# eladb3/SViT

Hardware: AMD Instinct MI355X
Metric: clips/sec (fwd+bwd) SViT 16x224^2 bf16 (higher is better)
Workload: dtype bf16; 1 GPU; SViT 16x224^2, 8 clips/GPU, 4 object tokens/frame, fwd+CE+bwd+clip+AdamW; global_batch=8, parallelism=dp1, ranks_seen=1, forced_dp=False, launch=hip-graph replay, input=fp32 clips, resident in the replayed step's input buffers, hip_library=svit_amd/lib/libsvit_hip.so

## Files before the change

### include/svit_hip.h

```cpp
#ifndef SVIT_HIP_H
#define SVIT_HIP_H
#include <stdint.h>
#ifdef __cplusplus
extern "C" {
#endif

#define SVIT_HEAD_DIM 96

int svit_version(void);
const char* svit_arch(void);

enum {
  SVIT_EPI_BF16 = 0,
  SVIT_EPI_GELU = 1,
  SVIT_EPI_RESID = 2,
  SVIT_EPI_F32 = 3,
  SVIT_EPI_DGELU = 4,
  SVIT_EPI_RELQ = 5
};
typedef struct {
  const void* A; int32_t lda;
  const void* W; int32_t ldw;
  const float* bias;
  void* out; int32_t ldo;
// ... 80 lines not shown
  int32_t stride_hw;
  int32_t mode;
  float eps;
  float out_scale;
  const void* relq_R; const int32_t* relq_map; int32_t relq_lpad; float relq_scale;
} svit_pool_args;
int svit_pool_ln_fwd(const svit_pool_args* a, void* stream);

typedef struct {
  const void* d_main; int32_t main_is_f32; int32_t ld_main;
  const void* d_res; const void* d_extra;
  const void* pre; const float* mean; const float* rstd; const float* gamma;
  void* dpre; float* dgamma; float* dbeta;
  int32_t B, heads, Nout;
  float* workspace; int64_t workspace_floats;
  int32_t main_parts; int64_t main_part_stride;
  int32_t extra_is_bf16;
} svit_pool_ln_bwd_args;
int svit_pool_ln_bwd(const svit_pool_ln_bwd_args* a, void* stream);
typedef struct {
  const void* dpre; const float* conv_w; void* dqkv; int32_t which;
  int32_t B, heads, T, H, W, n_obj, stride_hw;
} svit_pool_dgrad_args;
typedef struct {
  const void* dpre; const void* qkv; int32_t which; float* dw;
  int32_t B, heads, T, H, W, n_obj, stride_hw;
  float* workspace; int64_t workspace_floats;
} svit_pool_wgrad_args;
int svit_pool_ln_fwd_qkv(const svit_pool_args* args3, void* stream);
int svit_pool_weight_sel(const float* src_base, const int64_t* src_off, uint32_t* dst, int n_tables,
                         void* stream);
int svit_pool_ln_fwd_qkv_sel(const svit_pool_args* args3, const uint32_t* const* sel3, void* stream);
int svit_pool_ln_bwd_qkv(const svit_pool_ln_bwd_args* args3, void* stream);
#ifdef SVIT_DIAG_POOL_STREAMING
int svit_pool_conv_dgrad(const svit_pool_dgrad_args* a, void* stream);
int svit_pool_conv_wgrad(const svit_pool_wgrad_args* a, void* stream);
int svit_pool_conv_dgrad_qkv(const svit_pool_dgrad_args* args3, void* stream);
int svit_pool_conv_wgrad_qkv(const svit_pool_wgrad_args* args3, void* stream);
#endif
int svit_pool_conv_bwd_qkv(const svit_pool_dgrad_args* dgrad3, const svit_pool_wgrad_args* wgrad3,
                           void* stream);
int64_t svit_pool_conv_bwd_workspace(const svit_pool_dgrad_args* dgrad3);

typedef struct {
  void* qa; int32_t ld;
  const float* rel_h; const float* rel_w; const float* rel_t;
  const int32_t* idx_h; const int32_t* idx_w; const int32_t* idx_t;
  int32_t B, heads, qt, qh, qw, kt, kh, kw, n_obj;
  float inv_scale;
} svit_relq_args;
int svit_relpos_q_fwd(const svit_relq_args* a, void* stream);
typedef struct {
  const void* qa; const void* dqa; int32_t ld;
  const float* rel_h; const float* rel_w; const float* rel_t;
  const int32_t* idx_h; const int32_t* idx_w; const int32_t* idx_t;
  float* dq_extra;
  float* drel_h; float* drel_w; float* drel_t;
  int32_t rows_h, rows_w, rows_t;
  int32_t B, heads, qt, qh, qw, kt, kh, kw, n_obj;
  float inv_scale;
  float* workspace; int64_t workspace_floats;
} svit_relq_bwd_args;
int svit_relpos_q_bwd(const svit_relq_bwd_args* a, void* stream);
typedef struct {
  const void* P; int32_t ldp; void* qa; int32_t ld;
  const int32_t* idx_h; const int32_t* idx_w; const int32_t* idx_t;
  int32_t row_h, row_w, row_t;
  int32_t B, heads, qt, qh, qw, kt, kh, kw, n_obj;
  float inv_scale;
} svit_relq_gather_args;
int svit_relpos_gather(const svit_relq_gather_args* a, void* stream);
typedef struct {
  const void* dqa; int32_t ld; void* D; int32_t ldd;
  const int32_t* idx_h; const int32_t* idx_w; const int32_t* idx_t;
  int32_t off_h, off_w, off_t;
  int32_t B, heads, qt, qh, qw, kt, kh, kw, n_obj;
  float inv_scale;
} svit_relq_scatter_args;
int svit_relpos_scatter(const svit_relq_scatter_args* a, void* stream);

typedef struct {
  const void* qa; const void* ka; const void* v; void* ctx; float* lse2;
  int32_t B, heads, Nq, Nk, DA; float scale; int32_t bias_cols;
} svit_attn_fwd_args;
int svit_attn_fwd(const svit_attn_fwd_args* a, void* stream);
typedef struct {
  const void* qa; const void* ka; const void* v; const void* ctx; const void* dctx;
  const float* lse2; float* delta;
  void* dqa;
  float* dk; float* dv;
  int32_t B, heads, Nq, Nk, DA, q_splits; float scale;
  int32_t bias_cols;
  void* relD; int32_t relD_ld; const int32_t* relD_map; float relD_scale;
  const void* relR; float* relX;
} svit_attn_bwd_args;
int svit_attn_bwd(const svit_attn_bwd_args* a, void* stream);
int svit_attn_bwd_parts(const svit_attn_bwd_args* a);

int svit_maxpool_fwd(const float* x, float* y, uint8_t* idx, int B, int T, int H, int W,
                     int n_obj, int C, void* stream);
int svit_maxpool_bwd(const float* dy, const uint8_t* idx, float* dx, int B, int T, int H, int W,
                     int n_obj, int C, void* stream);
int svit_maxpool_bwd_bf16(const float* dy, const uint8_t* idx, void* dx_bf16, int B, int T, int H, int W,
                          int n_obj, int C, void* stream);

int svit_sumsq(const float* g, int64_t n, float* sumsq, float* workspace,
               int64_t workspace_floats, void* stream);
int svit_adamw_step(float* p, const float* g, float* m, float* v, int64_t n, const float* sumsq,
                    float max_norm, float lr, float beta1, float beta2, float eps, float wd,
                    int step, float grad_scale, void* stream);

typedef struct {
  float lr[2], weight_decay[2];
  float max_norm, clip_value, grad_scale, reserved;
} svit_step_host;
typedef struct {
  int64_t applied, skipped;
  int32_t consecutive, apply;
  float coef, bc1, bc2_sqrt, sumsq, grad_norm, reserved;
} svit_step_dev;

int svit_adamw_bias_table(float beta1, float beta2, float* table, int64_t capacity, int64_t* n_entries);

int svit_step_guard(const float* g, int64_t n, const svit_step_host* host_rec, svit_step_dev* dev_rec,
                    const float* bias_table, int64_t table_entries, float* workspace, int64_t workspace_floats,
                    void* stream);
int svit_adamw_step_guarded(float* p, const float* g, float* m, float* v, int64_t n, int64_t n_decay,
                            const svit_step_host* host_rec, const svit_step_dev* dev_rec, float beta1, float beta2,
                            float eps, void* stream);

typedef struct {
  const float* tokens; int32_t B, N, C, T, O;
  const float* keep;
  const float* w_proj; const float* b_proj; int32_t n_cls;
  const float* w_box; const float* b_box;
  const float* w_bce; const float* b_bce;
  const float* w_con; const float* b_con;
  float* logits; float* boxes; float* contact; float* xobj;
} svit_head_args;
int svit_head_fwd(const svit_head_args* a, void* stream);
typedef struct {
  svit_head_args f;
  const float* dlogits; const float* dboxes; const float* dcontact; const float* dxobj;
  float* dtokens;
  float* gw_proj; float* gb_proj; float* gw_box; float* gb_box; float* gw_bce; float* gb_bce; float* gw_con; float* gb_con;
  int32_t ordered;
} svit_head_bwd_args;
int svit_head_bwd(const svit_head_bwd_args* g, void* stream);

int svit_haog_loss(const float* pred, const float* tar, const float* contact,
                   const int64_t* contact_tar, float* losses, float* g_l1, float* g_bce,
                   float* g_giou, float* g_contact, int R, int Rc, void* stream);
int svit_haog_loss_bwd(const float* upstream, const float* g_l1, const float* g_bce,
                       const float* g_giou, const float* g_contact, float* dpred,
                       float* dcontact, int R, int Rc, void* stream);

int svit_ce_loss(const float* logits, const int64_t* labels, int B, int C, float* loss, float* dlogits, void* stream);
int svit_ce_loss_soft(const float* logits, const float* target, const int64_t* labels, const void* mix, float on,
                      float off, int B, int C, float* loss, float* dlogits, void* stream);
int svit_step_draws(uint64_t* state, const float* keep, int n_blocks, int per_block, float* scales,
                    int n_drop, float p_drop, float* drop, void* stream);

int svit_ensemble_update(const float* preds, const int64_t* labels, const int64_t* clip_ids,
                         int N, int C, int num_clips, int num_videos, int mode, int repeat,
                         float* video_preds, int64_t* video_labels, int64_t* clip_count,
                         int* err, void* stream);
int svit_topk_correct(const float* video_preds, const int64_t* video_labels, int V, int C,
                      const int* ks, int nk, int* counts, int* err, void* stream);
int svit_debug_set(int key, int val);
int svit_debug_set_tn(int step_us_x100, int atomic_tbs_x100);
int svit_debug_set_tn_tile(int mode);
int svit_debug_set_pool(int key, int val);
int svit_debug_pool_bwd_path(void);
int svit_attn_debug_set(int key, int val);
int svit_debug_reset(void);
#ifdef __cplusplus
}
// ... 3 lines not shown
```

### svit_amd/csrc/attn_bwd.hip

```cpp
#include <algorithm>
#include "attn_common.h"
#include "../../include/svit_hip.h"

#ifdef SVIT_ATTN_STAMPS
__device__ unsigned long long g_bwd_stamps[64];
extern "C" int svit_debug_attn_bwd_stamps(unsigned long long* host, int n) {
  return (int)hipMemcpyFromSymbol(host, HIP_SYMBOL(g_bwd_stamps), sizeof(unsigned long long) * n);
}
#define BSTAMP(slot)                                                                    \
  do {                                                                                  \
    __builtin_amdgcn_sched_barrier(0);                                                  \
    if (stamp_on) g_bwd_stamps[(slot)] = wall_clock64();                                \
    __builtin_amdgcn_sched_barrier(0);                                                  \
  } while (0)
#else
#define BSTAMP(slot) do {} while (0)
#endif

#ifndef SVIT_ATTN_QSTAGE
#define SVIT_ATTN_QSTAGE 1
#endif

namespace {
using namespace attn;
constexpr int KT = 64;
constexpr int QR = 64;
constexpr float LN2 = 0.6931471805599453f;

struct FragAddr {
  unsigned rowa[2], tra[2];
  __device__ __forceinline__ void init(unsigned base, int lane) {
    const int hh = lane >> 5, row = lane & 31, sw = (row >> 2) & 3;
    rowa[0] = base + row * 64 + 16 * ((0 + hh) ^ sw);
    rowa[1] = base + row * 64 + 16 * ((2 + hh) ^ sw);
    const int cg = (lane >> 4) & 1, i = lane & 15, q = i >> 2, pp = i & 3;
    const int r0 = 4 * hh, ch = 2 * cg + (pp >> 1);
    const unsigned tb = base + 8 * (pp & 1);
    tra[0] = tb + (r0 + q) * 64 + 16 * (ch ^ ((r0 >> 2) & 3));
    tra[1] = tb + (r0 + 8 + q) * 64 + 16 * (ch ^ (((r0 + 8) >> 2) & 3));
  }
};

template <int DA, int KSU>
__global__ __launch_bounds__(256, 2) void attn_bwd_dq_kernel(svit_attn_bwd_args a) {
#if __HIP_DEVICE_COMPILE__
  constexpr int NP = DA / 32;
  constexpr int K_BYTES = KT * DA * 2, V_BYTES = KT * HD * 2, STAGE = K_BYTES + V_BYTES;
  using KLoad = BufTile<KT, DA, 4>;
  using VLoad = BufTile<KT, HD, 4>;
  extern __shared__ __attribute__((aligned(16))) unsigned char smem[];
  const int tid = threadIdx.x, lane = tid & 63, wave = tid >> 6, hh = lane >> 5;
#ifdef SVIT_ATTN_STAMPS
  const bool stamp_on = blockIdx.x == 0 && blockIdx.y == 0 && tid == 0;
#endif
  BSTAMP(0);
  const int wgid = xcd_remap(blockIdx.y * gridDim.x + blockIdx.x, gridDim.x * gridDim.y);
  const int bh = wgid / gridDim.x, b = bh / a.heads, head = bh % a.heads;
  const int qtile = wgid % gridDim.x;
  const int q0 = qtile * 128 + wave * 32;
  const int qi = q0 + (lane & 31);
  const int qc = min(qi, a.Nq - 1);
  const bf16_t* qa = (const bf16_t*)a.qa + ((size_t)bh * a.Nq) * DA;
  const bf16_t* ka = (const bf16_t*)a.ka + ((size_t)bh * a.Nk) * DA;
  const bf16_t* vv = (const bf16_t*)a.v + ((size_t)bh * a.Nk) * HD;
  const bf16_t* dor = (const bf16_t*)a.dctx + ((size_t)b * a.Nq + qc) * a.heads * HD + head * HD;
  const float lse = a.lse2[(size_t)bh * a.Nq + qc];

  const int nt = (a.Nk + KT - 1) / KT;
  KLoad kload;
  VLoad vload;
  kload.init(DA, wave, lane);
  vload.init(HD, wave, lane);
  const auto krs = __builtin_amdgcn_make_buffer_rsrc((void*)ka, 0, a.Nk * DA * 2, 0x00020000);
  const auto vrs = __builtin_amdgcn_make_buffer_rsrc((void*)vv, 0, a.Nk * HD * 2, 0x00020000);
  auto issue = [&](int t) {
    unsigned char* st = smem + (t & 1) * STAGE;
    const unsigned k0 = (unsigned)t * KT;
    kload.issue_auto(krs, k0 * DA * 2u, DA, a.Nk - (int)k0, st, wave, lane);
    vload.issue_auto(vrs, k0 * HD * 2u, HD, a.Nk - (int)k0, st + K_BYTES, wave, lane);
  };
  BSTAMP(1);
  issue(0);
  BSTAMP(2);

  bf16x8_t qf[KSU], dof[6];
#pragma unroll
  for (int ks = 0; ks < 6; ++ks) dof[ks] = *(const bf16x8_t*)(dor + ks * 16 + hh * 8);
  using QStage = RowStage<DA>;
  if constexpr (SVIT_ATTN_QSTAGE != 0) {
    unsigned char* qreg = smem + STAGE + wave * QStage::BYTES;
    QStage::issue(qa, DA, q0, a.Nq, qreg, lane);
    wait_vmcnt<0>();
#pragma unroll
    for (int ks = 0; ks < KSU; ++ks) qf[ks] = QStage::frag(qreg, ks, lane);
  } else {
#pragma unroll
    for (int ks = 0; ks < KSU; ++ks) qf[ks] = *(const bf16x8_t*)(qa + (size_t)qc * DA + ks * 16 + hh * 8);
  }
  float dlt;
  {
    const bf16_t* orow = (const bf16_t*)a.ctx + ((size_t)b * a.Nq + qc) * a.heads * HD + head * HD;
    float part = 0.f;
#pragma unroll
    for (int ks = 0; ks < 6; ++ks) {
      const uint4 o = *(const uint4*)(orow + ks * 16 + hh * 8);
      const uint4 d = __builtin_bit_cast(uint4, dof[ks]);
      uint4 q = __builtin_bit_cast(uint4, qf[ks]);
      if (qc == 0) q = make_uint4(0, 0, 0, 0);
      part += lo_bf16(d.x) * (lo_bf16(o.x) - lo_bf16(q.x)) + hi_bf16(d.x) * (hi_bf16(o.x) - hi_bf16(q.x));
      part += lo_bf16(d.y) * (lo_bf16(o.y) - lo_bf16(q.y)) + hi_bf16(d.y) * (hi_bf16(o.y) - hi_bf16(q.y));
      part += lo_bf16(d.z) * (lo_bf16(o.z) - lo_bf16(q.z)) + hi_bf16(d.z) * (hi_bf16(o.z) - hi_bf16(q.z));
      part += lo_bf16(d.w) * (lo_bf16(o.w) - lo_bf16(q.w)) + hi_bf16(d.w) * (hi_bf16(o.w) - hi_bf16(q.w));
    }
    dlt = part + __shfl_xor(part, 32, 64);
    if (hh == 0 && qi < a.Nq) {
      float* sc = a.delta + (size_t)bh * a.Nq * 2;
      sc[qi] = -lse;
      sc[a.Nq + qi] = -dlt;
    }
  }

#pragma unroll
  for (int ks = 0; ks < KSU; ++ks) asm volatile("" : "+v"(qf[ks]));
#pragma unroll
  for (int ks = 0; ks < 6; ++ks) asm volatile("" : "+v"(dof[ks]));
  float lse_p = lse, dlt_p = dlt;
  asm volatile("" : "+v"(lse_p), "+v"(dlt_p));

  f32x16_t dq[NP];
#pragma unroll
  for (int j = 0; j < NP; ++j)
#pragma unroll
    for (int r = 0; r < 16; ++r) dq[j][r] = 0.f;

  FragAddr fa;
  fa.init((unsigned)(size_t)smem, lane);
  constexpr bool CINIT = DA == 128;
  f32x16_t s_init, dp_init;
#pragma unroll
  for (int r = 0; r < 16; ++r) { s_init[r] = CINIT ? -lse_p : 0.f; dp_init[r] = CINIT ? -dlt_p : 0.f; }

  static_prio(blockIdx.y * gridDim.x + blockIdx.x, wave, 4);
  BSTAMP(3);
  for (int t = 0; t < nt; ++t) {
// ... 147 lines not shown
    bf16_t vals[NV];
#pragma unroll
    for (int it = 0; it < NV; ++it) {
      const int e = it * 64 + lane, rl = e / EXTRA, j = e % EXTRA;
      vals[it] = *(const bf16_t*)(ost + rl * OROW + (96 + j) * 2);
    }
    asm volatile("s_waitcnt lgkmcnt(0)" ::: "memory");
    const int ldd = a.relD_ld, cpr = ldd >> 3;
    const int rpp = ldd <= 128 ? 32 : 8;
    bf16_t* Dg = (bf16_t*)a.relD + ((size_t)bh * a.Nq) * ldd;
    for (int r0 = 0; r0 < 32; r0 += rpp) {
      const int n16 = rpp * cpr;
      for (int i = lane; i < n16; i += 64) *(uint4*)(ost + i * 16) = make_uint4(0u, 0u, 0u, 0u);
      asm volatile("s_waitcnt lgkmcnt(0)" ::: "memory");
#pragma unroll
      for (int it = 0; it < NV; ++it) {
        const int e = it * 64 + lane, rl = e / EXTRA, j = e % EXTRA;
        if (rl >= r0 && rl < r0 + rpp && cols[it] >= 0)
          *(bf16_t*)(ost + ((rl - r0) * ldd + cols[it]) * 2) = f32_to_bf16(bf16_to_f32(vals[it]) * a.relD_scale);
      }
      asm volatile("s_waitcnt lgkmcnt(0)" ::: "memory");
      for (int i = lane; i < n16; i += 64) {
        const int rl = i / cpr, ch = i % cpr;
        if (q0 + r0 + rl < a.Nq)
          *(uint4*)(Dg + (size_t)(q0 + r0 + rl) * ldd + ch * 8) = *(const uint4*)(ost + i * 16);
      }
      if (a.relX && rpp == 32) {
        f32x16_t ex[3];
#pragma unroll
        for (int pb = 0; pb < 3; ++pb)
#pragma unroll
          for (int r = 0; r < 16; ++r) ex[pb][r] = 0.f;
        const bf16_t* R = (const bf16_t*)a.relR;
        for (int ks = 0; ks < ldd / 16; ++ks) {
          const bf16x8_t dfrag = *(const bf16x8_t*)(ost + ((lane & 31) * ldd + 16 * ks + 8 * hh) * 2);
#pragma unroll
          for (int pb = 0; pb < 3; ++pb) {
            const bf16x8_t rfrag = *(const bf16x8_t*)(R + (size_t)(pb * 32 + (lane & 31)) * ldd + 16 * ks + 8 * hh);
            ex[pb] = mfma32(rfrag, dfrag, ex[pb]);
          }
        }
        if (qi < a.Nq) {
          float* xr = a.relX + ((size_t)bh * a.Nq + qi) * HD;
#pragma unroll
          for (int pb = 0; pb < 3; ++pb)
#pragma unroll
            for (int g = 0; g < 4; ++g)
              *(float4*)(xr + pb * 32 + 8 * g + 4 * hh) =
                  make_float4(ex[pb][4 * g], ex[pb][4 * g + 1], ex[pb][4 * g + 2], ex[pb][4 * g + 3]);
        }
      }
      asm volatile("s_waitcnt lgkmcnt(0)" ::: "memory");
    }
  }
  BSTAMP(5);
#endif
}

template <int DA, int KSU, int NH>
__global__ __launch_bounds__(256 * NH, NH == 2 ? 1 : 2) void attn_bwd_dkv_kernel(svit_attn_bwd_args a,
                                                                                 int tiles_per_split) {
#if __HIP_DEVICE_COMPILE__
  constexpr int Q_BYTES = QR * DA * 2, O_BYTES = QR * HD * 2;
  constexpr int STAGE = Q_BYTES + O_BYTES + 2 * QR * 4;
  constexpr int NSTAGE = NH == 2 ? 3 : 2;
  constexpr int DR = DA == 160 ? 3 : 4, DT = DA == 160 ? 2 : 3;
  using QLoad = BufTile<QR, DA, 4 * NH>;
  using OLoad = BufTile<QR, HD, 4 * NH>;
  constexpr int PER_STAGE = QLoad::PER_WAVE + OLoad::PER_WAVE + 1;
  extern __shared__ __attribute__((aligned(16))) unsigned char smem[];
  const int tid = threadIdx.x, lane = tid & 63, wave = tid >> 6, hh = lane >> 5;
  const int kg = wave & 3, qh = wave >> 2;
#ifdef SVIT_ATTN_STAMPS
  const bool stamp_on = blockIdx.x == 0 && blockIdx.y == 0 && blockIdx.z == 0 && tid == 0;
#endif
  BSTAMP(32);
  const int wgid = xcd_remap((blockIdx.z * gridDim.y + blockIdx.y) * gridDim.x + blockIdx.x,
                             gridDim.x * gridDim.y * gridDim.z);
  const int bx = wgid % gridDim.x, by = (wgid / gridDim.x) % gridDim.y;
  const int bh = wgid / (gridDim.x * gridDim.y), b = bh / a.heads, head = bh % a.heads;
  const int key0 = bx * 128;
  const int ki = key0 + kg * 32 + (lane & 31);
  const int kc = min(ki, a.Nk - 1);
  const bf16_t* qa = (const bf16_t*)a.qa + ((size_t)bh * a.Nq) * DA;
  const bf16_t* ka = (const bf16_t*)a.ka + ((size_t)bh * a.Nk) * DA;
  const bf16_t* vv = (const bf16_t*)a.v + ((size_t)bh * a.Nk) * HD;
  const bf16_t* dob = (const bf16_t*)a.dctx + ((size_t)b * a.Nq) * a.heads * HD + head * HD;
  const float* sc_g = a.delta + (size_t)bh * a.Nq * 2;
  const int ldo = a.heads * HD;

  const int nqt = (a.Nq + QR - 1) / QR;
  const int t_begin = by * tiles_per_split;
  const int t_end = min(nqt, t_begin + tiles_per_split);
  QLoad qload;
  OLoad oload;
  qload.init(DA, wave, lane);
  oload.init(ldo, wave, lane);
  const auto qrs = __builtin_amdgcn_make_buffer_rsrc((void*)qa, 0, a.Nq * DA * 2, 0x00020000);
  const auto ors = __builtin_amdgcn_make_buffer_rsrc((void*)dob, 0, (a.Nq * ldo - head * HD) * 2, 0x00020000);
  auto issue = [&](int t) {
    unsigned char* st = smem + ((t - t_begin) % NSTAGE) * STAGE;
    const int q0 = t * QR;
    qload.issue_auto(qrs, (unsigned)q0 * DA * 2u, DA, a.Nq - q0, st, wave, lane);
    oload.issue_auto(ors, (unsigned)q0 * ldo * 2u, ldo, a.Nq - q0, st + Q_BYTES, wave, lane);
    const int part = wave & 1;
    const int qrow = min(q0 + lane, a.Nq - 1);
    __builtin_amdgcn_global_load_lds(
        (const __attribute__((address_space(1))) void*)(sc_g + (size_t)part * a.Nq + qrow),
        (__attribute__((address_space(3))) void*)(st + Q_BYTES + O_BYTES + part * 256), 4, 0, 0);
  };
  BSTAMP(33);
  if (t_begin < t_end) issue(t_begin);
  if (NSTAGE == 3 && t_begin + 1 < t_end) issue(t_begin + 1);
  BSTAMP(34);

  bf16x8_t kf[KSU], vf[6];
#pragma unroll
  for (int ks = 0; ks < KSU; ++ks) kf[ks] = *(const bf16x8_t*)(ka + (size_t)kc * DA + ks * 16 + hh * 8);
#pragma unroll
  for (int ks = 0; ks < 6; ++ks) vf[ks] = *(const bf16x8_t*)(vv + (size_t)kc * HD + ks * 16 + hh * 8);
#pragma unroll
  for (int ks = 0; ks < KSU; ++ks) asm volatile("" : "+v"(kf[ks]));
#pragma unroll
  for (int ks = 0; ks < 6; ++ks) asm volatile("" : "+v"(vf[ks]));

  f32x16_t dk[3], dv[3];
#pragma unroll
  for (int j = 0; j < 3; ++j)
#pragma unroll
    for (int r = 0; r < 16; ++r) { dk[j][r] = 0.f; dv[j][r] = 0.f; }

  BSTAMP(35);
  FragAddr fa;
  fa.init((unsigned)(size_t)smem + (NH == 2 ? qh * 2048 : 0), lane);
  const unsigned cba = (unsigned)(size_t)smem + Q_BYTES + O_BYTES + 16 * hh + (NH == 2 ? qh * 128 : 0);

  static_prio((blockIdx.z * gridDim.y + blockIdx.y) * gridDim.x + blockIdx.x, wave, 4 * NH);
  for (int t = t_begin; t < t_end; ++t) {
    if (t - t_begin < 4) BSTAMP(44 + 4 * (t - t_begin));
    if (NSTAGE == 3 && t + 1 < t_end) wait_vmcnt<PER_STAGE>();
    else wait_vmcnt<0>();
    if (t - t_begin < 4) BSTAMP(45 + 4 * (t - t_begin));
    __builtin_amdgcn_s_barrier();
    if (t - t_begin < 4) BSTAMP(46 + 4 * (t - t_begin));
    if (t + NSTAGE - 1 < t_end) issue(t + NSTAGE - 1);
    if (t - t_begin < 4) BSTAMP(47 + 4 * (t - t_begin));
    const unsigned so = ((t - t_begin) % NSTAGE) * STAGE;
    const unsigned ra[2] = {fa.rowa[0] + so, fa.rowa[1] + so};
    const unsigned ta[2] = {fa.tra[0] + so, fa.tra[1] + so};
    const unsigned ca = cba + so;
    static_for<0, (NH == 2 ? 1 : 2)>([&](auto HF) {
      constexpr int HB = NH == 2 ? 0 : decltype(HF)::value * 2048;
      constexpr int HC = NH == 2 ? 0 : decltype(HF)::value * 128;
      const int q0 = t * QR + (NH == 2 ? qh : decltype(HF)::value) * 32;
      f32x4_t cl[4], cd[4];
      static_for<0, 4>([&](auto G) {
        constexpr int g = decltype(G)::value;
        lds_read128f<HC + g * 32>(cl[g], ca);
        lds_read128f<HC + 256 + g * 32>(cd[g], ca);
      });
      RowStream<KSU + 6, DR> rs;
      auto rd = [&](auto J, bf16x8_t& d) {
        constexpr int j = decltype(J)::value;
        if constexpr (j < KSU) lds_read128<HB + (j >> 1) * 4096>(d, ra[j & 1]);
        else lds_read128<HB + Q_BYTES + ((j - KSU) >> 1) * 4096>(d, ra[(j - KSU) & 1]);
      };
// ... 103 lines not shown
    splits = (g_dkv_target + base - 1) / base;
    if (splits > nqt / 2) splits = nqt / 2;
  }
  if (splits > nqt) splits = nqt;
  if (splits < 1) splits = 1;
  const int tiles_per_split = (nqt + splits - 1) / splits;
  splits = (nqt + tiles_per_split - 1) / tiles_per_split;
  return {halves, splits, tiles_per_split};
}

template <int DA, int KSU>
int launch_bwd(const svit_attn_bwd_args& a, hipStream_t st) {
  static SvitOnce once_dq, once_kv, once_kv2;
  size_t lds_dq = 2 * (size_t)(KT * DA * 2 + KT * HD * 2);
  const size_t lds_dq_out = (size_t)4 * 32 * (DA * 2 + 16) + (size_t)4 * 32 * 128 * 2;
  if (lds_dq < lds_dq_out) lds_dq = lds_dq_out;
  lds_dq = std::max(lds_dq, (size_t)(KT * DA * 2 + KT * HD * 2) + 4 * (size_t)attn::RowStage<DA>::BYTES);
  const size_t stage = (size_t)(QR * DA * 2 + QR * HD * 2 + 2 * QR * 4);
  size_t lds_kv = 2 * stage, lds_kv2 = 3 * stage;
  const size_t lds_merge = (size_t)2 * 12 * 256 * 16;
  if (lds_kv2 < lds_merge) lds_kv2 = lds_merge;
  if (int rc = svit_max_lds_once(once_dq, (const void*)attn_bwd_dq_kernel<DA, KSU>, lds_dq)) return rc;
  if (int rc = svit_max_lds_once(once_kv, (const void*)attn_bwd_dkv_kernel<DA, KSU, 1>, lds_kv)) return rc;
  if (int rc = svit_max_lds_once(once_kv2, (const void*)attn_bwd_dkv_kernel<DA, KSU, 2>, lds_kv2)) return rc;
  const DkvPlan pl = dkv_plan(a);
  const int key_blocks = (a.Nk + 127) / 128;
  if (((uintptr_t)a.dk | (uintptr_t)a.dv) & 15) return SVIT_ERR_ALIGN;
  constexpr int skip = SVIT_DIAG_BWD_ONLY == 1 ? 2 : SVIT_DIAG_BWD_ONLY == 2 ? 1 : 0;
  if (!(skip & 1))
    hipLaunchKernelGGL((attn_bwd_dq_kernel<DA, KSU>), dim3((a.Nq + 127) / 128, a.B * a.heads), dim3(256),
                       lds_dq, st, a);
  SVIT_LAUNCH_CHECK();
  if (skip & 2) return SVIT_OK;
  if (pl.halves == 2)
    hipLaunchKernelGGL((attn_bwd_dkv_kernel<DA, KSU, 2>), dim3(key_blocks, pl.splits, a.B * a.heads), dim3(512),
                       lds_kv2, st, a, pl.tiles_per_split);
  else
    hipLaunchKernelGGL((attn_bwd_dkv_kernel<DA, KSU, 1>), dim3(key_blocks, pl.splits, a.B * a.heads), dim3(256),
                       lds_kv, st, a, pl.tiles_per_split);
  SVIT_LAUNCH_CHECK();
  return SVIT_OK;
}
}

static int check_bwd_args(const svit_attn_bwd_args* a) {
  if (!a) return SVIT_ERR_ARG;
  if (a->B <= 0 || a->heads <= 0 || a->Nq <= 0 || a->Nk <= 0) return SVIT_ERR_SHAPE;
  if (a->B * a->heads > 65535) return SVIT_ERR_SHAPE;
  if (a->DA != 128 && a->DA != 160) return SVIT_ERR_SHAPE;
  if (a->bias_cols < 0 || a->bias_cols > a->DA - 96) return SVIT_ERR_ARG;
  return SVIT_OK;
}

extern "C" int svit_attn_bwd_parts(const svit_attn_bwd_args* a) {
  if (int rc = check_bwd_args(a)) return rc;
  return dkv_plan(*a).splits;
}

extern "C" int svit_attn_bwd(const svit_attn_bwd_args* a, void* stream) {
  if (!a || !a->qa || !a->ka || !a->v || !a->ctx || !a->dctx || !a->lse2 || !a->delta || !a->dqa ||
      !a->dk || !a->dv)
    return SVIT_ERR_ARG;
  if (a->B <= 0 || a->heads <= 0 || a->Nq <= 0 || a->Nk <= 0) return SVIT_ERR_SHAPE;
  if (a->B * a->heads > 65535) return SVIT_ERR_SHAPE;
  if (a->DA != 128 && a->DA != 160) return SVIT_ERR_SHAPE;
  if (a->bias_cols < 0 || a->bias_cols > a->DA - 96) return SVIT_ERR_ARG;
  if (((uintptr_t)a->qa | (uintptr_t)a->ka | (uintptr_t)a->v | (uintptr_t)a->dctx | (uintptr_t)a->dqa) & 15)
    return SVIT_ERR_ALIGN;
  if (a->relD) {
    if (!a->relD_map || a->relD_ld <= 0 || a->relD_ld % 8 != 0 || a->relD_ld > 544) return SVIT_ERR_ARG;
    if ((uintptr_t)a->relD & 15) return SVIT_ERR_ALIGN;
    if (a->relX && (!a->relR || a->relD_ld > 128 || a->relD_ld % 16 != 0 ||
                    (((uintptr_t)a->relR | (uintptr_t)a->relX) & 15)))
      return SVIT_ERR_ARG;
    if (a->relR && !a->relX && (a->relD_ld > 128 || a->relD_ld % 16 != 0 || ((uintptr_t)a->relR & 15) ||
                                ((uintptr_t)a->relD_map & 15)))
      return SVIT_ERR_ARG;
  } else if (a->relX || a->relR) {
    return SVIT_ERR_ARG;
  }
  const int bias_cols = a->bias_cols > 0 ? a->bias_cols : a->DA - 96;
  const int ksu = 6 + (bias_cols + 15) / 16;
  hipStream_t st = (hipStream_t)stream;
  if (a->DA == 128) return ksu <= 7 ? launch_bwd<128, 7>(*a, st) : launch_bwd<128, 8>(*a, st);
  return ksu <= 9 ? launch_bwd<160, 9>(*a, st) : launch_bwd<160, 10>(*a, st);
}
```

### svit_amd/csrc/attn_common.h

```cpp
#pragma once
#include <type_traits>
#include "common.h"

namespace attn {

constexpr int HD = 96;

__device__ __forceinline__ int panel_byte(int rows, int row, int col8 ) {
  const int p = col8 >> 2, c = col8 & 3;
  return p * rows * 64 + row * 64 + 16 * (c ^ ((row >> 2) & 3));
}

template <int ROWS>
__device__ __forceinline__ bf16x8_t row_frag(const unsigned char* tile, int row0, int ks, int lane) {
  const int row = row0 + (lane & 31);
  return *(const bf16x8_t*)(tile + panel_byte(ROWS, row, 2 * ks + (lane >> 5)));
}

template <int ROWS>
__device__ __forceinline__ bf16x8_t tr_frag(const unsigned char* tile, int rbase, int panel,
                                            int lane) {
  const int hh = lane >> 5, cg = (lane >> 4) & 1, i = lane & 15, q = i >> 2, pp = i & 3;
  const int r0 = rbase + 4 * hh;
  const int ch = 2 * cg + (pp >> 1);
// ... 243 lines not shown
      voff[i] = (unsigned)(row * ld + panel * 32 + ch * 8) * 2u;
    }
  }
#if __HIP_DEVICE_COMPILE__
  template <typename RSRC>
  __device__ __forceinline__ void issue(RSRC rsrc, unsigned soff_bytes, unsigned char* tile, int wave) const {
#pragma unroll
    for (int i = 0; i < PER_WAVE; ++i) {
      int n = wave + i * NWAVES;
      if (n >= INSTRS) n = INSTRS - 1;
      __builtin_amdgcn_raw_ptr_buffer_load_lds(
          rsrc, (__attribute__((address_space(3))) void*)(tile + (n / RG) * ROWS * 64 + (n % RG) * 1024),
          16, voff[i], soff_bytes, 0, 0);
    }
  }
  template <typename RSRC>
  __device__ static __forceinline__ void issue_clamped(RSRC rsrc, unsigned soff_bytes, int ld, int valid_rows,
                                                       unsigned char* tile, int wave, int lane) {
#pragma unroll
    for (int i = 0; i < PER_WAVE; ++i) {
      int n = wave + i * NWAVES;
      if (n >= INSTRS) n = INSTRS - 1;
      const int panel = n / RG, rg = n % RG;
      const int row = rg * 16 + (lane >> 2);
      const int ch = (lane & 3) ^ ((row >> 2) & 3);
      const int grow = min(row, valid_rows - 1);
      __builtin_amdgcn_raw_ptr_buffer_load_lds(
          rsrc, (__attribute__((address_space(3))) void*)(tile + (n / RG) * ROWS * 64 + (n % RG) * 1024),
          16, (unsigned)(grow * ld + panel * 32 + ch * 8) * 2u, soff_bytes, 0, 0);
    }
  }
  template <typename RSRC>
  __device__ __forceinline__ void issue_auto(RSRC rsrc, unsigned soff_bytes, int ld, int valid_rows,
                                             unsigned char* tile, int wave, int lane) const {
    if (valid_rows >= ROWS) issue(rsrc, soff_bytes, tile, wave);
    else issue_clamped(rsrc, soff_bytes, ld, valid_rows, tile, wave, lane);
  }
#endif
};

template <int COLS>
struct RowStage {
  static constexpr int CPR = COLS / 8;
  static constexpr int RPP = 64 / CPR;
  static constexpr int PIECES = (32 + RPP - 1) / RPP;
  static constexpr int BYTES = PIECES * 1024;
  __device__ static __forceinline__ void issue(const bf16_t* __restrict__ base, size_t ld, int first, int nrows,
                                               unsigned char* region, int lane) {
    int rl = lane / CPR, c = lane % CPR;
    if (rl >= RPP) { rl = RPP - 1; c = 0; }
#pragma unroll
    for (int p = 0; p < PIECES; ++p) {
      const int r = min(p * RPP + rl, 31);
      const int g = (c + CPR - r % CPR) % CPR;
      const int row = min(first + r, nrows - 1);
      __builtin_amdgcn_global_load_lds(
          (const __attribute__((address_space(1))) void*)(base + (size_t)row * ld + g * 8),
          (__attribute__((address_space(3))) void*)(region + p * 1024), 16, 0, 0);
    }
  }
  __device__ static __forceinline__ bf16x8_t frag(const unsigned char* region, int ks, int lane) {
    const int r = lane & 31, g = 2 * ks + (lane >> 5);
    return *(const bf16x8_t*)(region + (r / RPP) * 1024 + (r % RPP) * (CPR * 16) + ((g + r) % CPR) * 16);
  }
};

#ifndef SVIT_ATTN_PRIO
#define SVIT_ATTN_PRIO 0
#endif
__device__ __forceinline__ void static_prio(int lin_wg, int wave, int nwaves) {
  bool hi = false;
  if (nwaves == 8) hi = (SVIT_ATTN_PRIO & 8) ? false : wave >= 4;
  else if ((SVIT_ATTN_PRIO & 7) == 1) hi = lin_wg & 1;
  else if ((SVIT_ATTN_PRIO & 7) == 2) hi = (lin_wg >> 3) & 1;
  else if ((SVIT_ATTN_PRIO & 7) == 3) hi = (lin_wg >> 8) & 1;
  if (SVIT_ATTN_PRIO != 0 && hi) __builtin_amdgcn_s_setprio(1);
}

template <int N>
__device__ __forceinline__ void wait_vmcnt() {
  asm volatile("s_waitcnt vmcnt(%0)" ::"n"(N) : "memory");
}

}


__device__ __forceinline__ int xcd_remap(int lin, int nwg) {
  const int xq = nwg >> 3, xr = nwg & 7, xcd = lin & 7;
  return (xcd < xr ? xcd * (xq + 1) : xr * (xq + 1) + (xcd - xr) * xq) + (lin >> 3);
}
```

### svit_amd/csrc/attn_fwd.hip

```cpp
#include <algorithm>
#include "attn_common.h"
#include "../../include/svit_hip.h"

#ifdef SVIT_ATTN_STAMPS
__device__ unsigned long long g_attn_stamps[8192];
extern "C" int svit_debug_attn_stamps(unsigned long long* host, int n) {
  return (int)hipMemcpyFromSymbol(host, HIP_SYMBOL(g_attn_stamps), sizeof(unsigned long long) * n);
}
#define STAMP(slot)                                                                     \
  do {                                                                                  \
    __builtin_amdgcn_sched_barrier(0);                                                  \
    if (stamp_on) g_attn_stamps[(slot)] = __builtin_readcyclecounter();                 \
    __builtin_amdgcn_sched_barrier(0);                                                  \
  } while (0)
#else
#define STAMP(slot) do {} while (0)
#endif

#ifndef SVIT_ATTN_ABL
#define SVIT_ATTN_ABL 0
#endif
#ifndef SVIT_ATTN_QSTAGE
#define SVIT_ATTN_QSTAGE 1
#endif

namespace {
using namespace attn;
constexpr int KT = 64;

__device__ __forceinline__ float other_half(float x) {
  const unsigned u = __float_as_uint(x);
  const auto r = __builtin_amdgcn_permlane32_swap(u, u, false, false);
  return __uint_as_float((threadIdx.x & 32) ? r[0] : r[1]);
}

template <int KSU, int NW, int NS>
__global__ __launch_bounds__(NW * 64, NW == 8 ? 1 : 2) void attn_fwd_kernel(svit_attn_fwd_args a) {
#if __HIP_DEVICE_COMPILE__
  constexpr int NP = (KSU + 1) / 2, KCOLS = NP * 32;
  constexpr int K_BYTES = KT * KCOLS * 2, V_BYTES = KT * HD * 2;
  constexpr int STAGE = K_BYTES + V_BYTES;
  using KLoad = BufTile<KT, KCOLS, NW>;
  using VLoad = BufTile<KT, HD, NW>;
  constexpr int PIECES = KLoad::PER_WAVE + VLoad::PER_WAVE;
  using QStage = RowStage<(KSU <= 8 ? 128 : 160)>;
  constexpr bool QSTAGE = (SVIT_ATTN_ABL & 1) == 0 && SVIT_ATTN_QSTAGE;
  extern __shared__ __attribute__((aligned(16))) unsigned char smem[];

  const int tid = threadIdx.x, lane = tid & 63, wave = tid >> 6, hh = lane >> 5;
#ifdef SVIT_ATTN_STAMPS
  if (blockIdx.x == 0 && blockIdx.y == 0 && tid == 0) g_attn_stamps[4] = __builtin_readcyclecounter();
#endif
  const int DA = a.DA;
  const int wgid = xcd_remap(blockIdx.y * gridDim.x + blockIdx.x, gridDim.x * gridDim.y);
  const int bh = wgid / gridDim.x, b = bh / a.heads, head = bh % a.heads;
  const int q0 = (wgid % gridDim.x) * (NW * 32) + wave * 32;
  const int qi = q0 + (lane & 31);
  const int qc = min(qi, a.Nq - 1);
  const bf16_t* qa = (const bf16_t*)a.qa + ((size_t)bh * a.Nq) * DA;
  const bf16_t* ka = (const bf16_t*)a.ka + ((size_t)bh * a.Nk) * DA;
  const bf16_t* vv = (const bf16_t*)a.v + ((size_t)bh * a.Nk) * HD;

  f32x16_t o[3], lacc, negm;
#pragma unroll
  for (int r = 0; r < 16; ++r) { lacc[r] = 0.f; negm[r] = 0.f; }
#pragma unroll
  for (int j = 0; j < 3; ++j)
#pragma unroll
    for (int r = 0; r < 16; ++r) o[j][r] = 0.f;
  bf16x8_t onesf;
#pragma unroll
  for (int e = 0; e < 8; ++e) onesf[e] = (lane & 31) == 0 ? (__bf16)1.0f : (__bf16)0.0f;
  float m_run = 0.f;

  const unsigned lds0 = (unsigned)(size_t)smem;
  unsigned kaddr0[2], vaddr0[2];
  {
    const int row = lane & 31, sw = (row >> 2) & 3;
    kaddr0[0] = lds0 + row * 64 + 16 * ((0 + hh) ^ sw);
    kaddr0[1] = lds0 + row * 64 + 16 * ((2 + hh) ^ sw);
    const int cg = (lane >> 4) & 1, i = lane & 15, q = i >> 2, pp = i & 3;
    const int r0 = 4 * hh, ch = 2 * cg + (pp >> 1);
    const unsigned vb = lds0 + K_BYTES + 8 * (pp & 1);
    vaddr0[0] = vb + (r0 + q) * 64 + 16 * (ch ^ ((r0 >> 2) & 3));
    vaddr0[1] = vb + (r0 + 8 + q) * 64 + 16 * (ch ^ (((r0 + 8) >> 2) & 3));
  }

#ifdef SVIT_ATTN_STAMPS
  const bool stamp_on = blockIdx.x == 0 && blockIdx.y == 0 && tid == 0;
  if (stamp_on) { g_attn_stamps[0] = __builtin_readcyclecounter(); g_attn_stamps[1] = wall_clock64(); }
#endif
  const int nt = (a.Nk + KT - 1) / KT;
  KLoad kload;
  VLoad vload;
  kload.init(DA, wave, lane);
  vload.init(HD, wave, lane);
  const auto krs = __builtin_amdgcn_make_buffer_rsrc((void*)ka, 0, a.Nk * DA * 2, 0x00020000);
  const auto vrs = __builtin_amdgcn_make_buffer_rsrc((void*)vv, 0, a.Nk * HD * 2, 0x00020000);
  auto issue = [&](int t) {
    if constexpr ((SVIT_ATTN_ABL & 8) != 0) return;
    unsigned char* st = smem + (t % NS) * STAGE;
    const unsigned k0 = (unsigned)t * KT;
    kload.issue_auto(krs, k0 * DA * 2u, DA, a.Nk - (int)k0, st, wave, lane);
    vload.issue_auto(vrs, k0 * HD * 2u, HD, a.Nk - (int)k0, st + K_BYTES, wave, lane);
  };
  issue(0);
  if (NS == 3 && nt > 1) issue(1);
  bf16x8_t qf[KSU];
  if constexpr (QSTAGE) {
    unsigned char* qreg = smem + (NS - 1) * STAGE + wave * QStage::BYTES;
    QStage::issue(qa, DA, q0, a.Nq, qreg, lane);
    wait_vmcnt<0>();
#pragma unroll
    for (int ks = 0; ks < KSU; ++ks) qf[ks] = QStage::frag(qreg, ks, lane);
  } else {
#pragma unroll
    for (int ks = 0; ks < KSU; ++ks) {
      if constexpr ((SVIT_ATTN_ABL & 1) != 0) {
        for (int e = 0; e < 8; ++e) qf[ks][e] = (__bf16)(0.01f * (float)(lane + ks));
      } else {
        qf[ks] = *(const bf16x8_t*)(qa + (size_t)qc * DA + ks * 16 + hh * 8);
      }
    }
  }
#pragma unroll
  for (int ks = 0; ks < KSU; ++ks) asm volatile("" : "+v"(qf[ks]));
  static_prio(blockIdx.y * gridDim.x + blockIdx.x, wave, NW);

  auto tile = [&](int t, auto HalfTag) {
    constexpr bool HALF = decltype(HalfTag)::value == 1;
    constexpr int NKB = HALF ? 1 : 2;
    if (NS == 3 && t + 1 < nt) wait_vmcnt<PIECES>();
    else wait_vmcnt<0>();
    STAMP(8 + t * 8 + 5);
    __builtin_amdgcn_s_barrier();
    STAMP(8 + t * 8 + 0);
    if (t + NS - 1 < nt) issue(t + NS - 1);
    STAMP(8 + t * 8 + 1);
    const unsigned so = (t % NS) * STAGE;
    const unsigned kaddr[2] = {kaddr0[0] + so, kaddr0[1] + so};
    const unsigned vaddr[2] = {vaddr0[0] + so, vaddr0[1] + so};
// ... 68 lines not shown
                            HALF ? acc_to_frag(s[0], 0) : acc_to_frag(s[1], 0),
                            HALF ? acc_to_frag(s[0], 1) : acc_to_frag(s[1], 1)};
    vs.run(rdv, [&](auto J, const bf16x8_t& f) {
      constexpr int i = decltype(J)::value, g = i / 3, j = i % 3;
      o[j] = mfma32(f, pf[g], o[j]);
      if constexpr (j == 2) lacc = mfma32(onesf, pf[g], lacc);
    });
    STAMP(8 + t * 8 + 4);
  };
  for (int t = 0; t + 1 < nt; ++t) tile(t, Int<0>{});
  if (a.Nk - (nt - 1) * KT > 32) tile(nt - 1, Int<0>{});
  else tile(nt - 1, Int<1>{});
#ifdef SVIT_ATTN_STAMPS
  if (stamp_on) { g_attn_stamps[2] = __builtin_readcyclecounter(); g_attn_stamps[3] = wall_clock64(); }
#endif

  uint4 qres[6];
#pragma unroll
  for (int it = 0; it < 6; ++it) {
    const int id = it * 64 + lane, row = id / 12, ch = id % 12;
    const int q = min(q0 + row, a.Nq - 1);
    if constexpr ((SVIT_ATTN_ABL & 2) != 0) qres[it] = make_uint4(0u, 0u, 0u, 0u);
    else qres[it] = *(const uint4*)(qa + (size_t)q * DA + ch * 8);
  }
  const float l_lo = __shfl(lacc[0], lane & 31, 64);
  const float inv = 1.f / l_lo;
  if (hh == 0 && qi < a.Nq) a.lse2[(size_t)bh * a.Nq + qi] = m_run + log2f(l_lo);
  __builtin_amdgcn_s_barrier();
  constexpr int OROW = 208;
  unsigned char* ost = smem + wave * (32 * OROW);
  {
    unsigned char* orow = ost + (lane & 31) * OROW;
#pragma unroll
    for (int j = 0; j < 3; ++j)
#pragma unroll
      for (int g = 0; g < 4; ++g) {
        const int dv = j * 32 + 8 * g + 4 * hh;
        uint2 pk;
        pk.x = pack_bf16x2(o[j][4 * g] * inv, o[j][4 * g + 1] * inv);
        pk.y = pack_bf16x2(o[j][4 * g + 2] * inv, o[j][4 * g + 3] * inv);
        *(uint2*)(orow + dv * 2) = pk;
      }
  }
#pragma unroll
  for (int it = 0; it < 6; ++it) {
    const int id = it * 64 + lane, row = id / 12, ch = id % 12;
    const int q = q0 + row;
    if (q < a.Nq) {
      uint4 ov = *(const uint4*)(ost + row * OROW + ch * 16);
      if (q > 0) {
        const uint4 qq = qres[it];
        ov.x = pack_bf16x2(lo_bf16(ov.x) + lo_bf16(qq.x), hi_bf16(ov.x) + hi_bf16(qq.x));
        ov.y = pack_bf16x2(lo_bf16(ov.y) + lo_bf16(qq.y), hi_bf16(ov.y) + hi_bf16(qq.y));
        ov.z = pack_bf16x2(lo_bf16(ov.z) + lo_bf16(qq.z), hi_bf16(ov.z) + hi_bf16(qq.z));
        ov.w = pack_bf16x2(lo_bf16(ov.w) + lo_bf16(qq.w), hi_bf16(ov.w) + hi_bf16(qq.w));
      }
      if constexpr ((SVIT_ATTN_ABL & 4) != 0) { if (ov.x == 0x12345678u && a.Nk < 0) a.lse2[0] = 1.f; }
      else *(uint4*)((bf16_t*)a.ctx + ((size_t)b * a.Nq + q) * a.heads * HD + head * HD + ch * 8) = ov;
    }
  }
#ifdef SVIT_ATTN_STAMPS
  __builtin_amdgcn_s_waitcnt(0);
  if (stamp_on) g_attn_stamps[5] = __builtin_readcyclecounter();
#endif
#endif
}


template <int KSU>
__global__ __launch_bounds__(256, 2) void attn_fwd_short_kernel(svit_attn_fwd_args a, int tiles_per_wg) {
#if __HIP_DEVICE_COMPILE__
  constexpr int NP = (KSU + 1) / 2, KCOLS = NP * 32;
  constexpr int K_BYTES = KT * KCOLS * 2, V_BYTES = KT * HD * 2, STAGE = K_BYTES + V_BYTES;
  using KLoad = BufTile<KT, KCOLS, 4>;
  using VLoad = BufTile<KT, HD, 4>;
  constexpr int OROW = 208;
  extern __shared__ __attribute__((aligned(16))) unsigned char smem[];
  const int tid = threadIdx.x, lane = tid & 63, wave = tid >> 6, hh = lane >> 5;
  const int DA = a.DA;
  const int wgid = xcd_remap(blockIdx.y * gridDim.x + blockIdx.x, gridDim.x * gridDim.y);
  const int bh = wgid / gridDim.x, b = bh / a.heads, head = bh % a.heads;
  const int ntiles = (a.Nq + 127) / 128;
  const int t_begin = (wgid % gridDim.x) * tiles_per_wg, t_end = min(ntiles, t_begin + tiles_per_wg);
  const bf16_t* qa = (const bf16_t*)a.qa + ((size_t)bh * a.Nq) * DA;
  const bf16_t* ka = (const bf16_t*)a.ka + ((size_t)bh * a.Nk) * DA;
  const bf16_t* vv = (const bf16_t*)a.v + ((size_t)bh * a.Nk) * HD;

  KLoad kload;
  VLoad vload;
  kload.init(DA, wave, lane);
  vload.init(HD, wave, lane);
  const auto krs = __builtin_amdgcn_make_buffer_rsrc((void*)ka, 0, a.Nk * DA * 2, 0x00020000);
  const auto vrs = __builtin_amdgcn_make_buffer_rsrc((void*)vv, 0, a.Nk * HD * 2, 0x00020000);
  kload.issue_auto(krs, 0u, DA, a.Nk, smem, wave, lane);
  vload.issue_auto(vrs, 0u, HD, a.Nk, smem + K_BYTES, wave, lane);
  bf16x8_t qn[KSU];
  auto load_q = [&](int tile) {
    const int qc = min(tile * 128 + wave * 32 + (lane & 31), a.Nq - 1);
#pragma unroll
    for (int ks = 0; ks < KSU; ++ks) qn[ks] = *(const bf16x8_t*)(qa + (size_t)qc * DA + ks * 16 + hh * 8);
  };
  load_q(t_begin);
  wait_vmcnt<0>();
  __builtin_amdgcn_s_barrier();

  bf16x8_t onesf;
#pragma unroll
  for (int e = 0; e < 8; ++e) onesf[e] = (lane & 31) == 0 ? (__bf16)1.0f : (__bf16)0.0f;
  const unsigned lds0 = (unsigned)(size_t)smem;
  unsigned kaddr[2], vaddr[2];
  {
    const int row = lane & 31, sw = (row >> 2) & 3;
    kaddr[0] = lds0 + row * 64 + 16 * ((0 + hh) ^ sw);
    kaddr[1] = lds0 + row * 64 + 16 * ((2 + hh) ^ sw);
    const int cg = (lane >> 4) & 1, i = lane & 15, q = i >> 2, pp = i & 3;
    const int r0 = 4 * hh, ch = 2 * cg + (pp >> 1);
    const unsigned vb = lds0 + K_BYTES + 8 * (pp & 1);
    vaddr[0] = vb + (r0 + q) * 64 + 16 * (ch ^ ((r0 >> 2) & 3));
    vaddr[1] = vb + (r0 + 8 + q) * 64 + 16 * (ch ^ (((r0 + 8) >> 2) & 3));
  }
  unsigned char* ost = smem + STAGE + wave * (32 * OROW);

  auto walk = [&](auto HalfTag) {
    constexpr bool HALF = decltype(HalfTag)::value == 1;
    constexpr int NKB = HALF ? 1 : 2;
    for (int tile = t_begin; tile < t_end; ++tile) {
      const int q0 = tile * 128 + wave * 32;
      if (q0 >= a.Nq) break;
      const int qi = q0 + (lane & 31);
      bf16x8_t qf[KSU];
#pragma unroll
      for (int ks = 0; ks < KSU; ++ks) qf[ks] = qn[ks];
#pragma unroll
      for (int ks = 0; ks < KSU; ++ks) asm volatile("" : "+v"(qf[ks]));
      if (tile + 1 < t_end) load_q(tile + 1);
      uint4 qres[6];
#pragma unroll
      for (int it = 0; it < 6; ++it) {
        const int id = it * 64 + lane, row = id / 12, ch = id % 12;
        const int q = min(q0 + row, a.Nq - 1);
        qres[it] = *(const uint4*)(qa + (size_t)q * DA + ch * 8);
      }
      TrStream<6 * NKB, 3> vs;
      auto rdv = [&](auto J, s16x4_t& lo, s16x4_t& hi) {
        constexpr int i = decltype(J)::value, g = i / 3, j = i % 3;
        lds_read_tr<g * 16 * 64 + j * KT * 64>(lo, vaddr[0]);
        lds_read_tr<g * 16 * 64 + j * KT * 64>(hi, vaddr[1]);
      };
      vs.prologue(rdv);
      f32x16_t s[2], zero;
#pragma unroll
      for (int r = 0; r < 16; ++r) zero[r] = 0.f;
      RowStream<KSU * NKB, 4> ks_;
      auto rdk = [&](auto J, bf16x8_t& d) {
        constexpr int j = decltype(J)::value, kb = j / KSU, ks = j % KSU;
        lds_read128<kb * 2048 + (ks >> 1) * KT * 64>(d, kaddr[ks & 1]);
      };
      ks_.prologue(rdk);
      ks_.run(rdk, [&](auto J, const bf16x8_t& f) {
        constexpr int j = decltype(J)::value, kb = j / KSU, ks = j % KSU;
        s[kb] = mfma32(f, qf[ks], ks == 0 ? zero : s[kb]);
      });
      if (KT > a.Nk) {
        asm volatile("; ragged key rows" ::: "memory");
#pragma unroll
        for (int kb = 0; kb < NKB; ++kb)
// ... 37 lines not shown
      const float l_lo = __shfl(lacc[0], lane & 31, 64);
      const float inv = 1.f / l_lo;
      if (hh == 0 && qi < a.Nq) a.lse2[(size_t)bh * a.Nq + qi] = mx + log2f(l_lo);
      {
        unsigned char* orow = ost + (lane & 31) * OROW;
#pragma unroll
        for (int j = 0; j < 3; ++j)
#pragma unroll
          for (int g = 0; g < 4; ++g) {
            const int dv = j * 32 + 8 * g + 4 * hh;
            uint2 pk;
            pk.x = pack_bf16x2(o[j][4 * g] * inv, o[j][4 * g + 1] * inv);
            pk.y = pack_bf16x2(o[j][4 * g + 2] * inv, o[j][4 * g + 3] * inv);
            *(uint2*)(orow + dv * 2) = pk;
          }
      }
#pragma unroll
      for (int it = 0; it < 6; ++it) {
        const int id = it * 64 + lane, row = id / 12, ch = id % 12;
        const int q = q0 + row;
        if (q < a.Nq) {
          uint4 ov = *(const uint4*)(ost + row * OROW + ch * 16);
          if (q > 0) {
            const uint4 qq = qres[it];
            ov.x = pack_bf16x2(lo_bf16(ov.x) + lo_bf16(qq.x), hi_bf16(ov.x) + hi_bf16(qq.x));
            ov.y = pack_bf16x2(lo_bf16(ov.y) + lo_bf16(qq.y), hi_bf16(ov.y) + hi_bf16(qq.y));
            ov.z = pack_bf16x2(lo_bf16(ov.z) + lo_bf16(qq.z), hi_bf16(ov.z) + hi_bf16(qq.z));
            ov.w = pack_bf16x2(lo_bf16(ov.w) + lo_bf16(qq.w), hi_bf16(ov.w) + hi_bf16(qq.w));
          }
          *(uint4*)((bf16_t*)a.ctx + ((size_t)b * a.Nq + q) * a.heads * HD + head * HD + ch * 8) = ov;
        }
      }
    }
  };
  if (a.Nk > 32) walk(Int<0>{});
  else walk(Int<1>{});
#endif
}

#ifndef SVIT_ATTN_SHORT_WGS
#define SVIT_ATTN_SHORT_WGS 512
#endif
template <int KSU>
int launch_short(const svit_attn_fwd_args& a, hipStream_t st) {
  constexpr int NP = (KSU + 1) / 2;
  const size_t lds = (size_t)(KT * NP * 32 * 2 + KT * HD * 2) + (size_t)4 * 32 * 208;
  static SvitOnce once;
  if (int rc = svit_max_lds_once(once, (const void*)attn_fwd_short_kernel<KSU>, lds)) return rc;
  constexpr int want = SVIT_ATTN_SHORT_WGS;
  const int ntiles = (a.Nq + 127) / 128, bh = a.B * a.heads;
  int chunks = (want + bh - 1) / bh;
  chunks = std::max(1, std::min(chunks, ntiles));
  const int per = (ntiles + chunks - 1) / chunks;
  chunks = (ntiles + per - 1) / per;
  hipLaunchKernelGGL((attn_fwd_short_kernel<KSU>), dim3(chunks, bh), dim3(256), lds, st, a, per);
  SVIT_LAUNCH_CHECK();
  return SVIT_OK;
}

template <int KSU, int NW, int NS>
int launch_cfg(const svit_attn_fwd_args& a, hipStream_t st) {
  constexpr int NP = (KSU + 1) / 2;
  const size_t stage = (size_t)(KT * NP * 32 * 2 + KT * HD * 2);
  size_t lds = NS * stage;
  const size_t lds_out = (size_t)NW * 32 * 208;
  if (lds < lds_out) lds = lds_out;
  if (SVIT_ATTN_QSTAGE)
    lds = std::max(lds, (NS - 1) * stage + NW * (size_t)attn::RowStage<(KSU <= 8 ? 128 : 160)>::BYTES);
  static SvitOnce once;
  if (int rc = svit_max_lds_once(once, (const void*)attn_fwd_kernel<KSU, NW, NS>, lds)) return rc;
  dim3 grid((a.Nq + NW * 32 - 1) / (NW * 32), a.B * a.heads);
  hipLaunchKernelGGL((attn_fwd_kernel<KSU, NW, NS>), grid, dim3(NW * 64), lds, st, a);
  SVIT_LAUNCH_CHECK();
  return SVIT_OK;
}

template <int KSU>
int launch_fwd(const svit_attn_fwd_args& a, hipStream_t st) {
  const long wg8 = (long)((a.Nq + 255) / 256) * a.B * a.heads;
  const bool wide = a.DA == 160 && wg8 >= 200;
  return wide ? launch_cfg<KSU, 8, 3>(a, st) : launch_cfg<KSU, 4, 2>(a, st);
}
}
extern "C" int svit_attn_fwd(const svit_attn_fwd_args* a, void* stream) {
  if (!a || !a->qa || !a->ka || !a->v || !a->ctx || !a->lse2) return SVIT_ERR_ARG;
  if (a->B <= 0 || a->heads <= 0 || a->Nq <= 0 || a->Nk <= 0) return SVIT_ERR_SHAPE;
  if (((uintptr_t)a->qa | (uintptr_t)a->ka | (uintptr_t)a->v | (uintptr_t)a->ctx) & 15)
    return SVIT_ERR_ALIGN;
  if (a->DA != 128 && a->DA != 160) return SVIT_ERR_SHAPE;
  if (a->bias_cols < 0 || a->bias_cols > a->DA - 96) return SVIT_ERR_ARG;
  const int extra = a->DA - 96;
  const int bias_cols = a->bias_cols > 0 ? a->bias_cols : extra;
  if (a->Nk <= KT && svit_knob(SVIT_K_ATTN_FWD_SHORT) != 0) {
    if (6 + (bias_cols + 15) / 16 == 7) return launch_short<7>(*a, (hipStream_t)stream);
    if (6 + (bias_cols + 15) / 16 == 8) return launch_short<8>(*a, (hipStream_t)stream);
  }
  switch (6 + (bias_cols + 15) / 16) {
    case 7: return launch_fwd<7>(*a, (hipStream_t)stream);
    case 8: return launch_fwd<8>(*a, (hipStream_t)stream);
    case 9: return launch_fwd<9>(*a, (hipStream_t)stream);
    case 10: return launch_fwd<10>(*a, (hipStream_t)stream);
  }
  return SVIT_ERR_SHAPE;
}
```

### svit_amd/csrc/common.h

```cpp
#pragma once
#include <hip/hip_runtime.h>
#include <stdint.h>

typedef uint16_t bf16_t;
typedef __bf16 bf16x8_t __attribute__((ext_vector_type(8)));
typedef __bf16 bf16x4_t __attribute__((ext_vector_type(4)));
typedef short s16x4_t __attribute__((ext_vector_type(4)));
typedef short s16x8_t __attribute__((ext_vector_type(8)));
typedef float f32x16_t __attribute__((ext_vector_type(16)));
typedef float f32x4_t __attribute__((ext_vector_type(4)));

#define SVIT_OK 0
#define SVIT_ERR_SHAPE (-2)
#define SVIT_ERR_ALIGN (-3)
#define SVIT_ERR_ARG (-4)

struct SvitOnce {
  unsigned long long mask;
};
static inline int svit_max_lds_once(SvitOnce& once, const void* fn, size_t bytes) {
  int dev = 0;
  if (hipGetDevice(&dev) != hipSuccess) dev = 0;
  const unsigned long long bit = 1ull << (dev & 63);
  if (__atomic_load_n(&once.mask, __ATOMIC_ACQUIRE) & bit) return 0;
  hipError_t e = hipFuncSetAttribute(fn, hipFuncAttributeMaxDynamicSharedMemorySize, (int)bytes);
  if (e != hipSuccess) return (int)e;
  __atomic_fetch_or(&once.mask, bit, __ATOMIC_RELEASE);
  return 0;
}

enum SvitKnob {
  SVIT_K_NT_STAGES = 0,
  SVIT_K_NT_CFG,
  SVIT_K_NT_BK,
  SVIT_K_TN_STEP_US_X100,
  SVIT_K_TN_ATOMIC_TBS_X100,
  SVIT_K_TN_TILE,
  SVIT_K_POOL_FWD,
  SVIT_K_POOL_BWD,
  SVIT_K_POOL_FWD_LARGE,
  SVIT_K_ATTN_DKV_FORM,
  SVIT_K_ATTN_FWD_SHORT,
  SVIT_K_POOL_FRAME,
  SVIT_K_COUNT
};
int svit_knob(int k);
int svit_knob_set(int k, int v);
void svit_knob_reset();

#define SVIT_LAUNCH_CHECK()                       \
  do {                                            \
    hipError_t e__ = hipGetLastError();           \
    if (e__ != hipSuccess) return (int)e__;       \
  } while (0)

__device__ __forceinline__ float bf16_to_f32(bf16_t v) {
  return __uint_as_float(((uint32_t)v) << 16);
}
__device__ __forceinline__ bf16_t f32_to_bf16(float f) {
  __bf16 b = (__bf16)f;
  return __builtin_bit_cast(bf16_t, b);
}
__device__ __forceinline__ uint32_t pack_bf16x2(float lo, float hi) {
  return (uint32_t)f32_to_bf16(lo) | ((uint32_t)f32_to_bf16(hi) << 16);
}
__device__ __forceinline__ float lo_bf16(uint32_t w) { return __uint_as_float(w << 16); }
__device__ __forceinline__ float hi_bf16(uint32_t w) { return __uint_as_float(w & 0xffff0000u); }

__device__ __forceinline__ float wave_sum(float v) {
#pragma unroll
  for (int o = 32; o > 0; o >>= 1) v += __shfl_xor(v, o, 64);
  return v;
}
__device__ __forceinline__ float wave_max(float v) {
#pragma unroll
  for (int o = 32; o > 0; o >>= 1) v = fmaxf(v, __shfl_xor(v, o, 64));
  return v;
}

__device__ __forceinline__ float fast_exp2(float x) { return __builtin_amdgcn_exp2f(x); }

__device__ __forceinline__ f32x16_t mfma32(bf16x8_t a, bf16x8_t b, f32x16_t c) {
  return __builtin_amdgcn_mfma_f32_32x32x16_bf16(a, b, c, 0, 0, 0);
}
__device__ __forceinline__ int acc_row(int r, int lane) {
  return (r & 3) + 8 * (r >> 2) + 4 * (lane >> 5);
}

typedef __attribute__((address_space(3))) s16x4_t lds_s16x4_t;
__device__ __forceinline__ s16x4_t lds_read_tr16(const void* p) {
  return __builtin_amdgcn_ds_read_tr16_b64_v4i16(
      (lds_s16x4_t*)(__attribute__((address_space(3))) void*)p);
}

__device__ __forceinline__ bf16x8_t make_bf16x8(s16x4_t lo, s16x4_t hi) {
  s16x8_t v = {lo[0], lo[1], lo[2], lo[3], hi[0], hi[1], hi[2], hi[3]};
  return __builtin_bit_cast(bf16x8_t, v);
}

__device__ __forceinline__ void gelu_parts(float x, float* cdf, float* pdf_scaled) {
  const float ax = fabsf(x) * 0.70710678118654752f;
  const float e = __expf(-ax * ax);
  const float t = __builtin_amdgcn_rcpf(1.0f + 0.3275911f * ax);
  const float poly = t * (0.254829592f + t * (-0.284496736f + t * (1.421413741f +
                     t * (-1.453152027f + t * 1.061405429f))));
  const float erf_abs = 1.0f - poly * e;
  const float erfv = x < 0.f ? -erf_abs : erf_abs;
  *cdf = 0.5f * (1.0f + erfv);
  *pdf_scaled = 0.39894228040143268f * e;
}
__device__ __forceinline__ float gelu_erf(float x) {
  float cdf, pdf;
  gelu_parts(x, &cdf, &pdf);
  return x * cdf;
}
__device__ __forceinline__ void gelu_fwd_grad(float x, float* y, float* dydx) {
#ifdef SVIT_DIAG_GELU_FREE
  *y = 0.5f * x; *dydx = 0.5f;
  return;
#endif
  float cdf, pdf;
  gelu_parts(x, &cdf, &pdf);
  *y = x * cdf;
  *dydx = cdf + x * pdf;
}
__device__ __forceinline__ float gelu_erf_grad(float x) {
// ... 25 lines not shown
```

### svit_amd/csrc/gemm_nt.hip

```cpp
#include "gemm_epilogue.h"
#include "attn_common.h"

namespace {

template <int BK>
__device__ __forceinline__ int nt_lds_off(int r, int ch) {
  if constexpr (BK == 32) return r * 64 + 16 * (ch ^ ((r >> 2) & 3));
  else return (r >> 4) * 2048 + (r & 7) * 256 + ((r >> 3) & 1) * 128 + 16 * (ch ^ (r & 7));
}

template <int N>
__device__ __forceinline__ void wait_vmcnt() {
  asm volatile("s_waitcnt vmcnt(%0)" ::"n"(N) : "memory");
}

template <int RB, int NB, int WAVES_M, int WAVES_N, int STAGES, int EPI, int BK2>
__global__ __launch_bounds__(WAVES_M* WAVES_N * 64, (WAVES_M * WAVES_N > 4 ? 1 : 2)) void
gemm_nt_v2_kernel(svit_gemm_args p) {
  constexpr int NT = WAVES_M * WAVES_N * 64;
  constexpr int BM = 32 * RB * WAVES_M, WN = 32 * NB, BN = WN * WAVES_N;
  constexpr int CPR = BK2 / 8;
  constexpr int RPR = NT / CPR;
  constexpr int ROWS = (BM + BN + RPR - 1) / RPR * RPR;
  constexpr int STAGE_BYTES = ROWS * BK2 * 2;
  constexpr int PER = ROWS * CPR / NT;
  extern __shared__ __attribute__((aligned(16))) unsigned char smem[];

  const int tid = threadIdx.x, lane = tid & 63, wave = tid >> 6;
  const int wm = wave / WAVES_N, wn = wave % WAVES_N;
  const int nwg = gridDim.x * gridDim.y, lin = blockIdx.y * gridDim.x + blockIdx.x;
  const int xq = nwg >> 3, xr = nwg & 7, xcd = lin & 7;
  const int wgid = (xcd < xr ? xcd * (xq + 1) : xr * (xq + 1) + (xcd - xr) * xq) + (lin >> 3);
  const int m0 = (wgid / gridDim.x) * BM, n0 = (wgid % gridDim.x) * BN;

  const bf16_t* src[PER];
#pragma unroll
  for (int i = 0; i < PER; ++i) {
    const int q = tid + i * NT;
    int row, ch;
    if constexpr (BK2 == 32) {
      row = q >> 2;
      ch = (q & 3) ^ ((row >> 2) & 3);
    } else {
      const int line = q >> 4;
      row = (line >> 3) * 16 + ((q >> 3) & 1) * 8 + (line & 7);
      ch = (q & 7) ^ (row & 7);
    }
    if (row < BM) {
      const int gr = min(m0 + row, p.M - 1);
      src[i] = (const bf16_t*)p.A + (size_t)gr * p.lda + ch * 8;
    } else {
      const int gr = min(n0 + row - BM, p.N - 1);
      src[i] = (const bf16_t*)p.W + (size_t)gr * p.ldw + ch * 8;
    }
  }
  auto issue = [&](int kt, int stage) {
    unsigned char* base = smem + stage * STAGE_BYTES + wave * 1024;
#pragma unroll
    for (int i = 0; i < PER; ++i)
      __builtin_amdgcn_global_load_lds(
          (const __attribute__((address_space(1))) void*)(src[i] + kt * BK2),
          (__attribute__((address_space(3))) void*)(base + i * (NT * 16)), 16, 0, 0);
  };

  f32x16_t acc[RB][NB];
#pragma unroll
  for (int i = 0; i < RB; ++i)
#pragma unroll
    for (int j = 0; j < NB; ++j)
#pragma unroll
      for (int r = 0; r < 16; ++r) acc[i][j][r] = 0.f;

  const int nk = p.K / BK2;
#pragma unroll
  for (int s = 0; s < STAGES - 1; ++s)
    if (s < nk) issue(s, s);

  const int a_row = wm * 32 * RB + (lane & 31);
  const int w_row = BM + wn * WN + (lane & 31);
  for (int kt = 0; kt < nk; ++kt) {
    if (kt + STAGES - 2 < nk) wait_vmcnt<(STAGES - 2) * PER>();
    else wait_vmcnt<0>();
    __builtin_amdgcn_s_barrier();
    if (kt + STAGES - 1 < nk) issue(kt + STAGES - 1, (kt + STAGES - 1) % STAGES);
    const unsigned char* st = smem + (kt % STAGES) * STAGE_BYTES;
    bf16x8_t af[BK2 / 16][RB], wf[BK2 / 16][NB];
#pragma unroll
    for (int ks = 0; ks < BK2 / 16; ++ks) {
      const int ch = 2 * ks + (lane >> 5);
#pragma unroll
      for (int i = 0; i < RB; ++i) {
        const int r = a_row + i * 32;
        af[ks][i] = *(const bf16x8_t*)(st + nt_lds_off<BK2>(r, ch));
      }
#pragma unroll
      for (int j = 0; j < NB; ++j) {
        const int r = w_row + j * 32;
        wf[ks][j] = *(const bf16x8_t*)(st + nt_lds_off<BK2>(r, ch));
      }
    }
    __builtin_amdgcn_sched_barrier(0);
#pragma unroll
    for (int ks = 0; ks < BK2 / 16; ++ks)
#pragma unroll
      for (int i = 0; i < RB; ++i)
#pragma unroll
        for (int j = 0; j < NB; ++j) acc[i][j] = mfma32(af[ks][i], wf[ks][j], acc[i][j]);
    __builtin_amdgcn_sched_barrier(0);
  }
  __syncthreads();
  nt_epilogue<RB, NB, EPI, true>(p, acc, smem, m0, n0, wm, wn, lane, wave);
}

template <int RB, int NB, int WAVES_M, int WAVES_N, int STAGES, int BK2 = 32>
int launch_v2(const svit_gemm_args& a, hipStream_t st) {
  constexpr int BM = 32 * RB * WAVES_M, BN = 32 * NB * WAVES_N;
  constexpr int NT = WAVES_M * WAVES_N * 64;
  constexpr int RPR = NT / (BK2 / 8);
  size_t lds = (size_t)STAGES * ((BM + BN + RPR - 1) / RPR * RPR) * BK2 * 2;
  const size_t lds_epi = (size_t)WAVES_M * WAVES_N * 16 * (32 * NB + 4) * sizeof(float);
  if (lds < lds_epi) lds = lds_epi;
  dim3 grid((a.N + BN - 1) / BN, (a.M + BM - 1) / BM);
  static SvitOnce once[6];
#define SVIT_V2_ATTR(E)                                                                              \
  if (int rc = svit_max_lds_once(once[E], (const void*)gemm_nt_v2_kernel<RB, NB, WAVES_M, WAVES_N, STAGES, E, BK2>, lds)) \
    return rc
  SVIT_V2_ATTR(SVIT_EPI_BF16); SVIT_V2_ATTR(SVIT_EPI_GELU); SVIT_V2_ATTR(SVIT_EPI_RESID);
  SVIT_V2_ATTR(SVIT_EPI_F32); SVIT_V2_ATTR(SVIT_EPI_DGELU); SVIT_V2_ATTR(SVIT_EPI_RELQ);
#undef SVIT_V2_ATTR
#define SVIT_V2_CASE(E)                                                                       \
  case E:                                                                                     \
    hipLaunchKernelGGL((gemm_nt_v2_kernel<RB, NB, WAVES_M, WAVES_N, STAGES, E, BK2>), grid, dim3(NT), \
                       lds, st, a);                                                           \
    break;
  switch (a.epilogue) {
    SVIT_V2_CASE(SVIT_EPI_BF16)
    SVIT_V2_CASE(SVIT_EPI_GELU)
    SVIT_V2_CASE(SVIT_EPI_RESID)
    SVIT_V2_CASE(SVIT_EPI_F32)
    SVIT_V2_CASE(SVIT_EPI_DGELU)
    SVIT_V2_CASE(SVIT_EPI_RELQ)
    default:
      return SVIT_ERR_ARG;
  }
#undef SVIT_V2_CASE
  SVIT_LAUNCH_CHECK();
  return SVIT_OK;
}

template <int NL, int BM, int BN, int STAGES>
__device__ __forceinline__ void nt_ring_loader(const svit_gemm_args& p, unsigned char* smem, int lw, int lane,
                                               int m0, int n0, int nk) {
  constexpr int PIECES = (BM + BN) / 8;
  constexpr int PER = (PIECES + NL - 1) / NL;
  constexpr int STAGE_BYTES = (BM + BN) * 128;
  const bf16_t* src[PER];
  auto piece_of = [&](int i) { return min(lw + NL * i, PIECES - 1); };
#pragma unroll
  for (int i = 0; i < PER; ++i) {
    const int q = piece_of(i) * 64 + lane, line = q >> 4;
    const int row = (line >> 3) * 16 + ((q >> 3) & 1) * 8 + (line & 7);
    const int ch = (q & 7) ^ (row & 7);
    if (row < BM) src[i] = (const bf16_t*)p.A + (size_t)min(m0 + row, p.M - 1) * p.lda + ch * 8;
    else src[i] = (const bf16_t*)p.W + (size_t)min(n0 + row - BM, p.N - 1) * p.ldw + ch * 8;
  }
  auto issue = [&](int kt) {
    unsigned char* st = smem + (kt % STAGES) * STAGE_BYTES;
#pragma unroll
    for (int i = 0; i < PER; ++i)
      __builtin_amdgcn_global_load_lds((const __attribute__((address_space(1))) void*)(src[i] + kt * 64),
                                       (__attribute__((address_space(3))) void*)(st + piece_of(i) * 1024), 16, 0, 0);
  };
#pragma unroll
  for (int s = 0; s < STAGES; ++s)
    if (s < nk) issue(s);
  for (int kt = 0; kt < nk; ++kt) {
    const int younger = (kt == 0 ? min(STAGES - 1, nk - 1) : min(kt + STAGES - 2, nk - 1) - kt);
    attn::static_for<0, STAGES>([&](auto Y) {
      if (younger == decltype(Y)::value) wait_vmcnt<decltype(Y)::value * PER>();
    });
    __builtin_amdgcn_s_barrier();
    if (kt >= 1 && kt - 1 + STAGES < nk) issue(kt - 1 + STAGES);
  }
}

template <int RB, int NB, int WAVES_M, int WAVES_N, int NL, int STAGES, int EPI>
__global__ __launch_bounds__((WAVES_M * WAVES_N + NL) * 64, 1) void gemm_nt_ring_kernel(svit_gemm_args p) {
  using attn::Int;
  constexpr int NC = WAVES_M * WAVES_N;
  constexpr int BM = 32 * RB * WAVES_M, WN = 32 * NB, BN = WN * WAVES_N;
  static_assert(BM % 16 == 0 && BN % 16 == 0, "a 1-KiB piece must not straddle A and W rows");
  constexpr int STAGE_BYTES = (BM + BN) * 128;
  extern __shared__ __attribute__((aligned(16))) unsigned char smem[];

  const int lane = threadIdx.x & 63;
  const int wave = __builtin_amdgcn_readfirstlane(threadIdx.x >> 6);
  const int nwg = gridDim.x * gridDim.y, lin = blockIdx.y * gridDim.x + blockIdx.x;
  const int xq = nwg >> 3, xr = nwg & 7, xcd = lin & 7;
  const int wgid = (xcd < xr ? xcd * (xq + 1) : xr * (xq + 1) + (xcd - xr) * xq) + (lin >> 3);
  const int m0 = (wgid / gridDim.x) * BM, n0 = (wgid % gridDim.x) * BN;
  const int nk = p.K / 64;

  if (wave >= NC) {
    nt_ring_loader<NL, BM, BN, STAGES>(p, smem, wave - NC, lane, m0, n0, nk);
    return;
  }

  const int wm = wave / WAVES_N, wn = wave % WAVES_N;
  f32x16_t acc[RB][NB];
#pragma unroll
  for (int i = 0; i < RB; ++i)
#pragma unroll
    for (int j = 0; j < NB; ++j)
#pragma unroll
      for (int r = 0; r < 16; ++r) acc[i][j][r] = 0.f;

  const int l31 = lane & 31, x7 = lane & 7;
  unsigned fa[4], fw[4];
#pragma unroll
  for (int ks = 0; ks < 4; ++ks) {
    const unsigned lp = (unsigned)((l31 >> 4) * 2048 + x7 * 256 + ((l31 >> 3) & 1) * 128 +
                                   32 * (ks ^ (x7 >> 1)) + 16 * ((lane >> 5) ^ (x7 & 1)));
    fa[ks] = (unsigned)(size_t)smem + lp + (unsigned)(wm * 2 * RB) * 2048u;
    fw[ks] = (unsigned)(size_t)smem + lp + (unsigned)((BM + wn * WN) / 16) * 2048u;
  }
  bf16x8_t fr[2][RB + NB];
  auto reads = [&](auto KS, auto BUF, unsigned so, auto HALF) {
    constexpr int ks = decltype(KS)::value, b = decltype(BUF)::value, h = decltype(HALF)::value;
    attn::static_for<0, RB + NB>([&](auto F) {
      constexpr int f = decltype(F)::value;
      if constexpr ((f / 2) == h) {
        if constexpr (f < RB) attn::lds_read128<f * 4096>(fr[b][f], fa[ks] + so);
        else attn::lds_read128<(f - RB) * 4096>(fr[b][f], fw[ks] + so);
      }
    });
  };
  constexpr int NH = (RB + NB + 1) / 2;
  auto release = [&](auto BUF) {
    constexpr int b = decltype(BUF)::value;
    attn::static_for<0, RB + NB>([&](auto F) { attn::lgkm_release1<0>(fr[b][decltype(F)::value]); });
  };
  auto substep = [&](auto BUF, auto NEXT_KS, unsigned next_so, bool do_reads) {
    constexpr int b = decltype(BUF)::value;
    attn::static_for<0, RB * NB>([&](auto Q) {
      constexpr int q = decltype(Q)::value, i = q / NB, j = q % NB;
      acc[i][j] = mfma32(fr[b][i], fr[b][RB + j], acc[i][j]);
      if constexpr (q < NH) {
        if (do_reads) reads(NEXT_KS, Int<1 - b>{}, next_so, Int<q>{});
      }
      __builtin_amdgcn_sched_barrier(0);
    });
  };

  __builtin_amdgcn_s_barrier();
  attn::static_for<0, NH>([&](auto H) { reads(Int<0>{}, Int<0>{}, 0u, H); });
  release(Int<0>{});
  for (int kt = 0; kt < nk; ++kt) {
    const unsigned so = (unsigned)((kt % STAGES) * STAGE_BYTES);
    const unsigned so_next = (unsigned)(((kt + 1) % STAGES) * STAGE_BYTES);
    const bool more = kt + 1 < nk;
    substep(Int<0>{}, Int<1>{}, so, true);
    release(Int<1>{});
    substep(Int<1>{}, Int<2>{}, so, true);
    release(Int<0>{});
    substep(Int<0>{}, Int<3>{}, so, true);
    release(Int<1>{});
    if (more) __builtin_amdgcn_s_barrier();
    substep(Int<1>{}, Int<0>{}, so_next, more);
    if (more) release(Int<0>{});
  }
  unsigned char* epi = smem + (nk >= 2 ? (nk - 2) % STAGES : 1) * STAGE_BYTES;
  nt_epilogue<RB, NB, EPI, true>(p, acc, epi, m0, n0, wm, wn, lane, wave);
}

template <int RB, int NB, int WAVES_M, int WAVES_N, int NL, int STAGES>
int launch_ring(const svit_gemm_args& a, hipStream_t st) {
  constexpr int BM = 32 * RB * WAVES_M, BN = 32 * NB * WAVES_N, NT = (WAVES_M * WAVES_N + NL) * 64;
  constexpr size_t lds = (size_t)STAGES * (BM + BN) * 128;
  static_assert((size_t)WAVES_M * WAVES_N * 16 * (32 * NB + 4) * sizeof(float) <= (size_t)(BM + BN) * 128, "epilogue staging fits a slot");
  static_assert(lds <= 160 * 1024, "LDS");
  dim3 grid((a.N + BN - 1) / BN, (a.M + BM - 1) / BM);
  static SvitOnce once[5];
#define SVIT_RING_ATTR(E)                                                                              \
  if (int rc = svit_max_lds_once(once[E], (const void*)gemm_nt_ring_kernel<RB, NB, WAVES_M, WAVES_N, NL, STAGES, E>, lds)) \
    return rc
  SVIT_RING_ATTR(SVIT_EPI_BF16); SVIT_RING_ATTR(SVIT_EPI_GELU); SVIT_RING_ATTR(SVIT_EPI_RESID);
  SVIT_RING_ATTR(SVIT_EPI_F32); SVIT_RING_ATTR(SVIT_EPI_DGELU);
#undef SVIT_RING_ATTR
#define SVIT_RING_CASE(E)                                                                       \
  case E:                                                                                       \
    hipLaunchKernelGGL((gemm_nt_ring_kernel<RB, NB, WAVES_M, WAVES_N, NL, STAGES, E>), grid, dim3(NT), lds, st, a); \
    break;
  switch (a.epilogue) {
    SVIT_RING_CASE(SVIT_EPI_BF16)
    SVIT_RING_CASE(SVIT_EPI_GELU)
    SVIT_RING_CASE(SVIT_EPI_RESID)
    SVIT_RING_CASE(SVIT_EPI_F32)
    SVIT_RING_CASE(SVIT_EPI_DGELU)
    default:
      return SVIT_ERR_ARG;
  }
#undef SVIT_RING_CASE
  SVIT_LAUNCH_CHECK();
  return SVIT_OK;
}
}

static void ring_choice(const svit_gemm_args& a, int* cfg, int* stages) {
  const long tm = (a.M + 127) / 128;
  const long t192 = a.N % 192 == 0 ? tm * (a.N / 192) : 0, t96 = tm * ((a.N + 95) / 96);
  constexpr int k_min5 = 1024, t_max6 = 256, s6 = 4;
  if (t96 <= t_max6 && a.K >= 768) { *cfg = 6, *stages = (t96 > 256 ? 2 : s6); return; }
  if (t192 >= 160 && a.N <= 768 && a.K >= k_min5) { *cfg = 5, *stages = 3; return; }
}

extern "C" int svit_gemm_nt(const svit_gemm_args* args, void* stream) {
  if (!args || !args->A || !args->W) return SVIT_ERR_ARG;
  const svit_gemm_args& a = *args;
  const bool relq = a.epilogue == SVIT_EPI_RELQ;
  if (!relq && !a.out) return SVIT_ERR_ARG;
  if (relq) {
    if (!a.relq_map || !a.relq_out || (a.relq_extra != 32 && a.relq_extra != 64) || a.relq_rows < 1 ||
        a.relq_ld < 96 + a.relq_extra || a.bias)
      return SVIT_ERR_ARG;
  }
  if (a.M <= 0 || a.N <= 0 || a.K <= 0 || a.K % 32 != 0 || a.N % 96 != 0) return SVIT_ERR_SHAPE;
  if (a.lda % 8 != 0 || a.ldw % 8 != 0 || a.lda < a.K || a.ldw < a.K || (!relq && a.ldo < a.N))
    return SVIT_ERR_ALIGN;
  if (((uintptr_t)a.A | (uintptr_t)a.W) & 15) return SVIT_ERR_ALIGN;
  if (!relq && (a.ldo % 4 != 0 || ((uintptr_t)a.out & 15))) return SVIT_ERR_ALIGN;
  if (a.bias && ((uintptr_t)a.bias & 15)) return SVIT_ERR_ALIGN;
  if (a.aux && (a.ldaux % 4 != 0 || ((uintptr_t)a.aux & 15))) return SVIT_ERR_ALIGN;
  if (a.out2 && (a.ldo2 % 4 != 0 || ((uintptr_t)a.out2 & 15))) return SVIT_ERR_ALIGN;
  if ((a.epilogue == SVIT_EPI_RESID || a.epilogue == SVIT_EPI_DGELU) && !a.aux) return SVIT_ERR_ARG;
  if (a.epilogue == SVIT_EPI_RESID && a.row_scale && a.rows_per_sample <= 0) return SVIT_ERR_ARG;
  hipStream_t st = (hipStream_t)stream;
  const int force_raw = svit_knob(SVIT_K_NT_CFG), force_stages = svit_knob(SVIT_K_NT_STAGES);
  const bool no_ring = force_raw == 8 || svit_knob(SVIT_K_NT_BK) != 0;
  const int force_cfg = force_raw == 8 ? -1 : force_raw;
  if (a.K % 64 == 0 && !relq && ((force_cfg < 0 && !no_ring) || (force_cfg >= 5 && force_cfg <= 7))) {
    int cfg = force_cfg, rs = force_stages;
    if (cfg < 0) ring_choice(a, &cfg, &rs);
    if (cfg >= 5) {
      if (!rs) rs = 3;
#define SVIT_RING_PICK(RB, NB, WM, WN)                                         \
  do {                                                                         \
    if (rs == 2) return launch_ring<RB, NB, WM, WN, 4, 2>(a, st);              \
    if (rs == 3) return launch_ring<RB, NB, WM, WN, 4, 3>(a, st);              \
    return launch_ring<RB, NB, WM, WN, 4, 4>(a, st);                           \
  } while (0)
      if (cfg == 5) SVIT_RING_PICK(2, 3, 2, 2);
      if (cfg == 6) SVIT_RING_PICK(1, 3, 4, 1);
      SVIT_RING_PICK(2, 2, 2, 2);
#undef SVIT_RING_PICK
    }
  }
  bool big = a.N % 192 == 0 && (long)((a.M + 127) / 128) * (a.N / 192) >= 256;
  if (force_cfg == 0 && a.N % 192 == 0) big = true;
  if (force_cfg == 2) big = false;
  const int stages = force_stages ? force_stages : (a.K >= 2048 ? 4 : 2);
  bool sq = a.N % 128 == 0 && a.N >= 1024 && a.K <= 512 &&
            (long)((a.M + 127) / 128) * (a.N / 128) <= 2048;
  if (force_cfg == 4) sq = a.N % 128 == 0;
  else if (force_cfg >= 0) sq = false;
  const int force_bk = svit_knob(SVIT_K_NT_BK);
  bool bk64 = a.K % 64 == 0 && a.N <= 768 && a.K >= 384;
  if (force_bk) bk64 = force_bk == 64 && a.K % 64 == 0;
  if (bk64 && force_cfg < 0 && !force_stages) return launch_v2<1, 3, 4, 1, 2, 64>(a, st);
#define SVIT_NT_PICK(RB, NB, WM, WN)                                           \
  do {                                                                         \
    if (bk64) {                                                                \
      if (stages == 2) return launch_v2<RB, NB, WM, WN, 2, 64>(a, st);         \
      if (stages == 3) return launch_v2<RB, NB, WM, WN, 3, 64>(a, st);         \
      return launch_v2<RB, NB, WM, WN, 4, 64>(a, st);                          \
    }                                                                          \
    if (stages == 2) return launch_v2<RB, NB, WM, WN, 2, 32>(a, st);           \
    if (stages == 3) return launch_v2<RB, NB, WM, WN, 3, 32>(a, st);           \
    return launch_v2<RB, NB, WM, WN, 4, 32>(a, st);                            \
  } while (0)
  {
    constexpr int one_round = 1;
    const long t160 = a.N % 256 == 0 ? (long)((a.M + 159) / 160) * (a.N / 256) : 0;
    const long t192 = a.N % 192 == 0 ? (long)((a.M + 191) / 192) * (a.N / 192) : 0;
    const long t128 = (long)((a.M + 127) / 128) * ((a.N + 191) / 192);
    const bool auto_ok = force_cfg < 0 && one_round && !force_stages && !force_bk && a.K <= 512 && t128 > 512;
    if (force_cfg == 9 || (auto_ok && t160 > 256 && t160 <= 512)) {
      if (a.N % 256 == 0) return launch_v2<5, 2, 1, 4, 2, 32>(a, st);
    }
    if (force_cfg == 10 || (auto_ok && t192 > 256 && t192 <= 512)) {
      if (a.N % 192 == 0) return launch_v2<3, 3, 2, 2, 2, 32>(a, st);
    }
  }
  if (sq) SVIT_NT_PICK(2, 2, 2, 2);
  if (big) SVIT_NT_PICK(2, 3, 2, 2);
  SVIT_NT_PICK(1, 3, 4, 1);
#undef SVIT_NT_PICK
}
```

### svit_amd/csrc/misc.hip

```cpp
#include <mutex>
#include <unordered_map>
#include "common.h"
#include "../../include/svit_hip.h"

namespace {

__global__ void cast_kernel(const float* __restrict__ src, bf16_t* __restrict__ dst, int64_t n) {
  const int64_t stride = (int64_t)gridDim.x * blockDim.x * 8;
  for (int64_t i = ((int64_t)blockIdx.x * blockDim.x + threadIdx.x) * 8; i < n; i += stride) {
    if (i + 8 <= n) {
      const float4 a = *(const float4*)(src + i), b = *(const float4*)(src + i + 4);
      uint4 o;
      o.x = pack_bf16x2(a.x, a.y); o.y = pack_bf16x2(a.z, a.w);
      o.z = pack_bf16x2(b.x, b.y); o.w = pack_bf16x2(b.z, b.w);
      *(uint4*)(dst + i) = o;
    } else {
      for (int64_t j = i; j < n; ++j) dst[j] = f32_to_bf16(src[j]);
    }
  }
}

__global__ void transpose_cast_kernel(const float* __restrict__ src_base,
                                      bf16_t* __restrict__ dst_base,
                                      const int64_t* __restrict__ table, int n_mats) {
// ... 463 lines not shown
  const float cv = h->clip_value;
  const float lr0 = h->lr[0], lr1 = h->lr[1], wd0 = h->weight_decay[0], wd1 = h->weight_decay[1];
  const int64_t n4 = n >> 2;
  const int64_t stride = (int64_t)gridDim.x * blockDim.x;
  for (int64_t q = (int64_t)blockIdx.x * blockDim.x + threadIdx.x; q < n4; q += stride) {
    const int64_t i = q * 4;
    float4 P = ((const float4*)p)[q], M = ((const float4*)m)[q], V = ((const float4*)v)[q];
    const float4 G = ((const float4*)g)[q];
    const bool d0 = i < n_decay, d1 = i + 1 < n_decay, d2 = i + 2 < n_decay, d3 = i + 3 < n_decay;
    adamw_guarded_update<CLAMP>(P.x, G.x, M.x, V.x, coef, cv, d0 ? lr0 : lr1, d0 ? wd0 : wd1, b1, b2, eps, bc1, bc2_sqrt);
    adamw_guarded_update<CLAMP>(P.y, G.y, M.y, V.y, coef, cv, d1 ? lr0 : lr1, d1 ? wd0 : wd1, b1, b2, eps, bc1, bc2_sqrt);
    adamw_guarded_update<CLAMP>(P.z, G.z, M.z, V.z, coef, cv, d2 ? lr0 : lr1, d2 ? wd0 : wd1, b1, b2, eps, bc1, bc2_sqrt);
    adamw_guarded_update<CLAMP>(P.w, G.w, M.w, V.w, coef, cv, d3 ? lr0 : lr1, d3 ? wd0 : wd1, b1, b2, eps, bc1, bc2_sqrt);
    ((float4*)p)[q] = P; ((float4*)m)[q] = M; ((float4*)v)[q] = V;
  }
  const int64_t i = n4 * 4 + threadIdx.x;
  if (blockIdx.x == 0 && i < n) {
    const bool dec = i < n_decay;
    float pw = p[i], mo = m[i], va = v[i];
    adamw_guarded_update<CLAMP>(pw, g[i], mo, va, coef, cv, dec ? lr0 : lr1, dec ? wd0 : wd1, b1, b2, eps, bc1, bc2_sqrt);
    p[i] = pw; m[i] = mo; v[i] = va;
  }
}

__global__ __launch_bounds__(256) void adamw_guarded_kernel(float* __restrict__ p, const float* __restrict__ g,
                                                            float* __restrict__ m, float* __restrict__ v, int64_t n,
                                                            int64_t n_decay, const svit_step_host* __restrict__ h,
                                                            const svit_step_dev* __restrict__ d, float b1, float b2,
                                                            float eps) {
  if (d->apply == 0) return;
  const float coef = d->coef, bc1 = d->bc1, bc2_sqrt = d->bc2_sqrt;
  if (h->clip_value > 0.f) adamw_guarded_range<true>(p, g, m, v, n, n_decay, h, coef, bc1, bc2_sqrt, b1, b2, eps);
  else adamw_guarded_range<false>(p, g, m, v, n, n_decay, h, coef, bc1, bc2_sqrt, b1, b2, eps);
}

inline unsigned grid_for(int64_t work_items, int block, unsigned cap = 8192) {
  int64_t b = (work_items + block - 1) / block;
  if (b < 1) b = 1;
  if (b > cap) b = cap;
  return (unsigned)b;
}
__global__ __launch_bounds__(128) void table_interp_kernel(const float* __restrict__ M, int J, const float* __restrict__ T,
                                                           float* __restrict__ out32, bf16_t* __restrict__ out16) {
  const int r = blockIdx.x, c = threadIdx.x;
  if (c >= 96) return;
  const float* m = M + (size_t)r * J;
  float acc = 0.f;
#pragma unroll 8
  for (int j = 0; j < J; ++j) acc += m[j] * T[(size_t)j * 96 + c];
  if (out32) out32[(size_t)r * 96 + c] = acc;
  if (out16) out16[(size_t)r * 96 + c] = f32_to_bf16(acc);
}
__global__ __launch_bounds__(128) void table_interp_batched_kernel(const svit_table_interp_job* __restrict__ jobs) {
  const svit_table_interp_job j = jobs[blockIdx.y];
  const int r = blockIdx.x, c = threadIdx.x;
  if (r >= j.rows || c >= 96) return;
  const float* m = j.M + (size_t)r * j.J;
  float acc = 0.f;
#pragma unroll 8
  for (int k = 0; k < j.J; ++k) acc += m[k] * j.tables[(size_t)k * 96 + c];
  if (j.out32) j.out32[(size_t)r * 96 + c] = acc;
  if (j.out16) ((bf16_t*)j.out16)[(size_t)r * 96 + c] = f32_to_bf16(acc);
}
}

extern "C" int svit_version(void) { return 1; }

extern "C" int svit_table_interp_batched(const svit_table_interp_job* jobs_dev, int n_jobs, int max_rows, void* stream) {
  if (!jobs_dev || n_jobs <= 0 || n_jobs > 65535 || max_rows <= 0) return SVIT_ERR_ARG;
  hipLaunchKernelGGL(table_interp_batched_kernel, dim3(max_rows, n_jobs), dim3(128), 0, (hipStream_t)stream, jobs_dev);
  SVIT_LAUNCH_CHECK();
  return SVIT_OK;
}

extern "C" int svit_table_interp(const float* M, int rows, int J, const float* tables, float* out32, void* out16, void* stream) {
  if (!M || !tables || (!out32 && !out16) || rows <= 0 || J <= 0) return SVIT_ERR_ARG;
  hipLaunchKernelGGL(table_interp_kernel, dim3(rows), dim3(128), 0, (hipStream_t)stream, M, J, tables, out32, (bf16_t*)out16);
  SVIT_LAUNCH_CHECK();
  return SVIT_OK;
}

static const int k_knob_default[SVIT_K_COUNT] = {
     0,  -1,  0,  85,  75,  2,
     2,  1,  1,  0,  1,  2};
static int g_knob[SVIT_K_COUNT] = {0, -1, 0, 85, 75, 2, 2, 1, 1, 0, 1, 2};
int svit_knob(int k) { return __atomic_load_n(&g_knob[k], __ATOMIC_RELAXED); }
int svit_knob_set(int k, int v) {
  if (k < 0 || k >= SVIT_K_COUNT) return SVIT_ERR_ARG;
  __atomic_store_n(&g_knob[k], v, __ATOMIC_RELAXED);
  return SVIT_OK;
}
void svit_knob_reset() {
  for (int k = 0; k < SVIT_K_COUNT; ++k) __atomic_store_n(&g_knob[k], k_knob_default[k], __ATOMIC_RELAXED);
}
extern "C" int svit_debug_set(int key, int val) {
  if (key == 0) return (val == 0 || (val >= 2 && val <= 4)) ? svit_knob_set(SVIT_K_NT_STAGES, val) : SVIT_ERR_ARG;
  if (key == 1) return (val >= -1 && val <= 10) ? svit_knob_set(SVIT_K_NT_CFG, val) : SVIT_ERR_ARG;
  if (key == 2) return (val == 0 || val == 32 || val == 64) ? svit_knob_set(SVIT_K_NT_BK, val) : SVIT_ERR_ARG;
  return SVIT_ERR_ARG;
}
extern "C" int svit_debug_set_tn(int step_us_x100, int atomic_tbs_x100) {
  if (step_us_x100 > 0) svit_knob_set(SVIT_K_TN_STEP_US_X100, step_us_x100);
  if (atomic_tbs_x100 > 0) svit_knob_set(SVIT_K_TN_ATOMIC_TBS_X100, atomic_tbs_x100);
  return SVIT_OK;
}
extern "C" int svit_debug_set_tn_tile(int mode) {
  return (mode >= 0 && mode <= 3) ? svit_knob_set(SVIT_K_TN_TILE, mode) : SVIT_ERR_ARG;
}
extern "C" int svit_debug_set_pool(int key, int val) {
  if (key == 0) return (val >= 0 && val <= 3) ? svit_knob_set(SVIT_K_POOL_FWD, val) : SVIT_ERR_ARG;
  if (key == 1) return (val == 0 || val == 1) ? svit_knob_set(SVIT_K_POOL_BWD, val) : SVIT_ERR_ARG;
  if (key == 2) return (val == 0 || val == 1) ? svit_knob_set(SVIT_K_POOL_FWD_LARGE, val) : SVIT_ERR_ARG;
  if (key == 3) return (val >= 0 && val <= 2) ? svit_knob_set(SVIT_K_POOL_FRAME, val) : SVIT_ERR_ARG;
  return SVIT_ERR_ARG;
}
extern "C" int svit_attn_debug_set(int key, int val) {
  if (key == 0) return (val >= 0 && val <= 2) ? svit_knob_set(SVIT_K_ATTN_DKV_FORM, val) : SVIT_ERR_ARG;
  if (key == 3) return (val == 0 || val == 1) ? svit_knob_set(SVIT_K_ATTN_FWD_SHORT, val) : SVIT_ERR_ARG;
  return SVIT_ERR_ARG;
}
extern "C" int svit_debug_reset(void) { svit_knob_reset(); return SVIT_OK; }
extern "C" const char* svit_arch(void) { return "gfx950"; }

extern "C" int svit_cast_f32_bf16(const float* src, void* dst, int64_t n, void* stream) {
  if (!src || !dst || n <= 0) return SVIT_ERR_ARG;
  if (((uintptr_t)src | (uintptr_t)dst) & 15) return SVIT_ERR_ALIGN;
  hipLaunchKernelGGL(cast_kernel, dim3(grid_for((n + 7) / 8, 256)), dim3(256), 0,
                     (hipStream_t)stream, src, (bf16_t*)dst, n);
  SVIT_LAUNCH_CHECK();
  return SVIT_OK;
}

extern "C" int svit_transpose_cast_batched(const float* src_base, void* dst_base,
                                           const int64_t* table, int n_mats, int max_tiles,
                                           void* stream) {
  if (!src_base || !dst_base || !table || n_mats <= 0) return SVIT_ERR_ARG;
  int gx = max_tiles < 1 ? 1 : (max_tiles > 256 ? 256 : max_tiles);
  hipLaunchKernelGGL(transpose_cast_kernel, dim3(gx, n_mats), dim3(256), 0, (hipStream_t)stream,
                     src_base, (bf16_t*)dst_base, table, n_mats);
  SVIT_LAUNCH_CHECK();
  return SVIT_OK;
}


extern "C" int svit_transpose_bf16_batched(const void* src_base, void* dst_base, const int64_t* table,
                                           int n_mats, int max_tiles, void* stream) {
  if (!src_base || !dst_base || !table || n_mats <= 0) return SVIT_ERR_ARG;
  if (((uintptr_t)src_base | (uintptr_t)dst_base) & 15) return SVIT_ERR_ALIGN;
  int gx = max_tiles < 1 ? 1 : (max_tiles > 256 ? 256 : max_tiles);
  hipLaunchKernelGGL(transpose_bf16_kernel, dim3(gx, n_mats), dim3(256), 0, (hipStream_t)stream,
                     (const bf16_t*)src_base, (bf16_t*)dst_base, table, n_mats);
  SVIT_LAUNCH_CHECK();
  return SVIT_OK;
}

extern "C" int svit_scale_cast(const float* src, void* dst, const float* row_scale,
                               int rows_per_sample, int64_t rows, int cols, int gather_L,
                               int gather_N, int gather_off, void* stream) {
  if (!src || !dst || rows <= 0 || cols <= 0 || cols % 4 != 0) return SVIT_ERR_ARG;
  if (row_scale && rows_per_sample <= 0) return SVIT_ERR_ARG;
  if (gather_L < 0 || (gather_L > 0 && (gather_N < gather_L || gather_off < 0))) return SVIT_ERR_ARG;
  hipLaunchKernelGGL(scale_cast_kernel, dim3(grid_for(rows * (cols / 4), 256)), dim3(256), 0,
                     (hipStream_t)stream, src, (bf16_t*)dst, row_scale, rows_per_sample, rows,
                     cols, gather_L, gather_N, gather_off);
  SVIT_LAUNCH_CHECK();
  return SVIT_OK;
}

extern "C" int svit_pad_cast_rows(const float* src, void* dst, int R, int C, int ldd, void* stream) {
  if (!src || !dst || R <= 0 || C <= 0 || ldd < C) return SVIT_ERR_ARG;
  hipLaunchKernelGGL(pad_cast_rows_kernel, dim3(grid_for((int64_t)R * ldd, 256)), dim3(256), 0,
                     (hipStream_t)stream, src, (bf16_t*)dst, R, C, ldd);
  SVIT_LAUNCH_CHECK();
  return SVIT_OK;
}

extern "C" int svit_im2col_patch(const float* video, void* cols, int B, int T, int H, int W,
                                 void* stream) {
  if (!video || !cols || B <= 0 || T <= 0 || H <= 0 || W <= 0) return SVIT_ERR_ARG;
  const int To = (T + 2 - 3) / 2 + 1, Ho = (H + 6 - 7) / 4 + 1, Wo = (W + 6 - 7) / 4 + 1;
  hipLaunchKernelGGL(im2col_patch_kernel, dim3((unsigned)(B * To * Ho)), dim3(256), 0,
// ... 224 lines not shown
```

### svit_amd/engine.py

```python
import math

import torch

from . import arch, hip, ops
from .input import U8Clips

HD = arch.HEAD_DIM
F32, BF16 = torch.float32, torch.bfloat16
SCALE = HD ** -0.5
LOG2E = 1.4426950408889634
K_SCALE = SCALE * LOG2E


def _align(n, a=8):
    return (n + a - 1) // a * a


class FlatParams:

    def __init__(self, shapes, decay_of, device, rank_of):
        names = list(shapes)
        depth = 1 + max([int(n.split(".")[1]) for n in names if n.startswith("blocks.")] or [0])
        ranks = {n: rank_of(n, depth) for n in names}
        order = sorted(names, key=lambda n: (not decay_of(n, shapes[n]), ranks[n]))
# ... 203 lines not shown
        if jobs is not None:
            ops.table_interp_batched(jobs, max_rows)
        self._interp_out = outs

    def _relq_map(self, blk, q_thw, k_thw, idx, rows_off, n_obj, extra):
        key = (blk.index, q_thw, k_thw, tuple(rows_off), n_obj, extra)
        m = self._relq_cache.get(key)
        if m is None:
            qt, qh, qw = q_thw
            kt, kh, kw = k_thw
            ih, iw, it = (t.cpu().view(n, k) for t, n, k in zip(idx, (qh, qw, qt), (kh, kw, kt)))
            Lq = qt * qh * qw
            body = torch.full((qt, qh, qw, extra), -1, dtype=torch.int32)
            body[..., :kh] = (rows_off[0] + ih).view(1, qh, 1, kh)
            body[..., kh:kh + kw] = (rows_off[1] + iw).view(1, 1, qw, kw)
            body[..., kh + kw:kh + kw + kt] = (rows_off[2] + it).view(qt, 1, 1, kt)
            m = torch.full((1 + Lq + n_obj, extra), -1, dtype=torch.int32)
            m[1:1 + Lq] = body.view(Lq, extra)
            m = m.contiguous().to(self.dev)
            self._relq_cache[key] = m
        return m

    def _tables(self, pre, mats):
        names = (pre + "attn.rel_pos_h", pre + "attn.rel_pos_w", pre + "attn.rel_pos_t")
        out = []
        for n, m in zip(names, mats):
            t = self.flat.p(n)
            out.append(t if m is None else (m @ t).contiguous())
        return out

    def forward(self, video, drop_scales=None, save=True):
        plan, f = self.plan, self.flat
        if isinstance(video, U8Clips):
            B, _, Tx = video.shape[:3]
            cols, (To, Ho, Wo) = ops.im2col_patch_u8(video)
        else:
            if video.dim() == 4:
                video = video.unsqueeze(2)
            video = video.contiguous().to(F32)
            B, _, Tx = video.shape[:3]
            cols, (To, Ho, Wo) = ops.im2col_patch(video)
        T = plan.num_frames // plan.patch_stride[0] if Tx > 1 else Tx
        if To != T:
            raise hip.SvitHipError("clip has %d frames but cfg.DATA.NUM_FRAMES=%d" % (Tx, plan.num_frames))
        L, n_obj, C = To * Ho * Wo, Tx * plan.objects, plan.embed_dim
        N = 1 + L + n_obj
        x = torch.empty((B, N, C), device=self.dev, dtype=F32)
        ops.gemm_nt(cols, self.patch_w16, f.p("patch_embed.proj.bias"), hip.EPI_F32,
                    out=x.view(B * N, C), remap=(L, N, 1))
        ops.fill_special_tokens(x, f.p("cls_token"), f.p("object_queries"),
                                f.p("pos_embed_temporal"), L, Tx, plan.objects, Tx > 1)
        st = {"B": B, "Tx": Tx, "n_obj": n_obj, "L0": L, "cols": cols if save else None,
              "blocks": []}
        thw = (T, Ho, Wo)
        self._interp_tables(thw, save)
        hip.mark("stem")
        for blk in plan.blocks:
            ds = drop_scales[blk.index] if drop_scales is not None else None
            x, thw, sv = self._block_fwd(blk, x, thw, n_obj, ds, save)
            st["blocks"].append(sv)
            hip.mark("fwd%d" % blk.index)
        y16, y32, mean, rstd = ops.layernorm_fwd(x, f.p("norm.weight"), f.p("norm.bias"),
                                                 want_f32=True, want_bf16=False, save_stats=save)
        st.update(x_last=x if save else None, mean=mean, rstd=rstd, thw=thw)
        self._interp_out = {}
        return y32, st

    def _block_fwd(self, blk, x, thw, n_obj, ds, save):
        f = self.flat
        pre = "blocks.%d." % blk.index
        B, N, C = x.shape
        Co, h = blk.dim_out, blk.heads
        sq, skv = blk.stride_q[1], blk.stride_kv[1]
        q_thw = (thw[0], arch.pooled(thw[1], sq), arch.pooled(thw[2], sq))
        k_thw = (thw[0], arch.pooled(thw[1], skv), arch.pooled(thw[2], skv))
        Nq = 1 + q_thw[0] * q_thw[1] * q_thw[2] + n_obj
        J = k_thw[0] + k_thw[1] + k_thw[2]
        DA = HD + 32 if J <= 32 else HD + 64
        if J > 64:
            raise hip.SvitHipError("key grid %s too large for the in-MFMA rel-pos bias" % (k_thw,))
        xn, _, mean1, rstd1 = ops.layernorm_fwd(x, f.p(pre + "norm1.weight"), f.p(pre + "norm1.bias"),
                                                save_stats=save)
        xn2d = xn.view(B * N, C)
        qkv = ops.gemm_nt(xn2d, f.w(pre + "attn.qkv.weight"), f.p(pre + "attn.qkv.bias"), hip.EPI_BF16)
        idx, mats, mcat, need = self._rel(blk, q_thw, k_thw)
        if mcat is None:
            tabs = self._tables(pre, mats)
            rcat, rows_off = f.rel_cat(pre)
        else:
            if blk.index in self._interp_out:
                r32, rcat = self._interp_out[blk.index]
            else:
                r32, rcat = ops.table_interp(mcat, f.rel_tables32(pre), want_f32=save)
            rows_off = (0, need[0], need[0] + need[1])
            tabs = None if r32 is None else [r32[rows_off[0]:rows_off[0] + need[0]], r32[rows_off[1]:rows_off[1] + need[1]],
                                             r32[rows_off[2]:rows_off[2] + need[2]]]
        pools = ops.pool_ln_fwd_qkv(
            qkv, [f.p(pre + "attn.pool_%s.weight" % r).view(HD, 27) for r in "qkv"],
            [f.p(pre + "attn.norm_%s.weight" % r) for r in "qkv"],
            [f.p(pre + "attn.norm_%s.bias" % r) for r in "qkv"],
            B, h, thw, n_obj, (sq, skv, skv), (DA, DA, HD), (0, 1, 0), save=save, out_scales=(1.0, K_SCALE, 1.0),
            sels=f.sels(pre) if (thw[1] * thw[2] >= f.TILED_MIN_PLANE or thw[1] * thw[2] <= f.SLAB_MAX_PLANE)
            else None,
            relq=(rcat.contiguous(), self._relq_map(blk, q_thw, k_thw, idx, rows_off, n_obj, DA - HD), LOG2E))
        qa, ka, v = pools[0][0], pools[1][0], pools[2][0]
        ctx, lse2 = ops.attn_fwd(qa, ka, v, SCALE, bias_cols=J)
        pool_idx = None
        if blk.has_proj:
            skip = ops.gemm_nt(xn2d, f.w(pre + "proj.weight"), f.p(pre + "proj.bias"), hip.EPI_F32)
            skip = skip.view(B, N, Co)
        else:
            skip = x
        if blk.pools_q:
            skip, pool_idx = ops.maxpool_fwd(skip, thw, n_obj)
        dpa, dpm = ds if ds is not None else (None, None)
        x1 = ops.gemm_nt(ctx.view(B * Nq, Co), f.w(pre + "attn.proj.weight"), f.p(pre + "attn.proj.bias"),
                         hip.EPI_RESID, aux=skip.view(B * Nq, Co), row_scale=dpa, rows_per_sample=Nq)
        x1 = x1.view(B, Nq, Co)
        xn2, _, mean2, rstd2 = ops.layernorm_fwd(x1, f.p(pre + "norm2.weight"), f.p(pre + "norm2.bias"),
                                                 save_stats=save)
        act, dact = ops.gemm_nt(xn2.view(B * Nq, Co), f.w(pre + "mlp.fc1.weight"),
                                f.p(pre + "mlp.fc1.bias"), hip.EPI_GELU, save=save)
        x2 = ops.gemm_nt(act, f.w(pre + "mlp.fc2.weight"), f.p(pre + "mlp.fc2.bias"), hip.EPI_RESID,
                         aux=x1.view(B * Nq, Co), row_scale=dpm, rows_per_sample=Nq).view(B, Nq, Co)
        sv = None
        if save:
            sv = dict(x=x, thw=thw, q_thw=q_thw, k_thw=k_thw, mean1=mean1, rstd1=rstd1, xn=xn2d,
                      qkv=qkv, pools=pools, tabs=tabs, idx=idx, mats=mats, ctx=ctx, lse2=lse2,
                      pool_idx=pool_idx, x1=x1, mean2=mean2, rstd2=rstd2, xn2=xn2, act=act,
                      dact=dact, dpa=dpa, dpm=dpm, Nq=Nq)
        return x2, q_thw, sv

    def backward(self, st, dy, on_ready=None, ready_ranks=None):
        def ready(rank):
            if on_ready is not None:
                if ready_ranks is None or rank in ready_ranks:
                    ops.reduce_flush()
                    self._flush_tn()
                    self._join()
                on_ready(rank)
        plan, f = self.plan, self.flat
        depth = len(plan.blocks)
        last = st["blocks"][depth - 1]
        dx, dx16 = ops.layernorm_bwd(dy.contiguous(), st["x_last"], f.p("norm.weight"), st["mean"],
                                     st["rstd"], f.g("norm.weight"), f.g("norm.bias"),
                                     want_bf16=True, row_scale=last["dpm"],
                                     rows_per_sample=st["x_last"].shape[1])
        ready(0)
        hip.mark("bwd_norm")
        for blk in reversed(plan.blocks):
            below = st["blocks"][blk.index - 1] if blk.index > 0 else None
            try:
                G = self.RED_GROUP
                dx, dx16 = self._block_bwd(blk, st["blocks"][blk.index], dx, dx16, st["n_obj"], below,
                                           red_begin=blk.index % G == G - 1 or blk.index == depth - 1,
                                           red_end=blk.index % G == 0, red_slot=blk.index % G)
            except BaseException:
                ops.reduce_reset()
                self._tn = []
                raise
            hip.mark("bwd%d" % blk.index)
            ready(1 + (depth - 1 - blk.index))
        B, Tx, L, O, C = st["B"], st["Tx"], st["L0"], plan.objects, plan.embed_dim
        ops.special_token_grads(dx, f.g("cls_token"), f.g("object_queries"),
                                f.g("pos_embed_temporal") if Tx > 1 else None, L, Tx, O, Tx > 1)
        dtok = ops.scale_cast(dx, gather=(L, 1))
        self._gemm_tn(dtok, st["cols"], f.g("patch_embed.proj.weight").view(C, 441), f.g("patch_embed.proj.bias"))
        self._flush_tn()
        self._join()
        ready(depth + 1)

    def _rws(self, key):
        a, b = self._red_regions[key]
        o = self._red_slot * 18 * 1024 * 1024
        return self._red_ws[o + a:o + b]

    def _wgrad_ws(self, B, h, thw, n_obj, strides):
        key = (B, h, tuple(thw), n_obj, tuple(strides))
        need = self._wgrad_need.get(key)
        if need is None:
            need = self._wgrad_need[key] = ops.pool_conv_bwd_workspace(B, h, thw, n_obj, strides)
        ws = self._rws("wgrad")
        if need <= ws.numel():
            return ws
        big = self._wgrad_big.get(self._red_slot)
        if big is None or big.numel() < need:
            big = self._wgrad_big[self._red_slot] = torch.empty(need, device=self.dev, dtype=F32)
        return big

    def _fork(self, fn, keep):
        if not self.overlap_wgrad:
            fn()
            return
        if self._capture_fork is not None:
            self._capture_fork(fn)
            self._side_active = True
            return
        main = torch.cuda.current_stream(self.dev)
        if self._side is None:
            self._side = torch.cuda.Stream(device=self.dev)
        self._side.wait_stream(main)
        with torch.cuda.stream(self._side):
            fn()
        self._side_keep.append(keep)
        self._side_active = True

    def _join(self):
        if self._side_active and self._capture_join is not None:
            self._capture_join()
            self._side_active = False
            return
        if self._side_active:
            torch.cuda.current_stream(self.dev).wait_stream(self._side)
            self._side_keep.clear()
            self._side_active = False

    def _flush_tn(self, force=True):
        if not force and len(self._tn) <= 8:
            return
        q, self._tn = self._tn, []
        if not q:
            return
        det = self.deterministic
        if self.reproducible and not det:
            self._fork(lambda: ops.gemm_tn_grouped_slab(q, tag="tn_slab_queue"), q)
            return
        self._fork(lambda: ops.gemm_tn_grouped(q, ordered=det), q)

    def _gemm_tn(self, a, b, dw, dbias=None):
        if self.deterministic:
            ops.gemm_tn(a, b, dw, splits=1, dbias=dbias)
        elif self.reproducible:
            ops.gemm_tn_grouped_slab([(a, b, dw, dbias)], tag="tn_slab_main")
        else:
            ops.gemm_tn(a, b, dw, splits=0, dbias=dbias)

    def _linear_bwd(self, dy16, x16, wname, bname, need_dx, out=None, accumulate=False,
                    epilogue=hip.EPI_F32, aux=None):
        f = self.flat
        self._tn.append((dy16, x16, f.g(wname), f.g(bname)))
        if not need_dx:
            return None
        return ops.gemm_nt(dy16, f.wt(wname), None, epilogue, out=out, aux=aux, accumulate=accumulate)

    def _block_bwd(self, blk, sv, dx2, dy, n_obj, below, red_begin=True, red_end=True, red_slot=0):
        f = self.flat
        pre = "blocks.%d." % blk.index
        B, Nq, Co = dx2.shape
        x = sv["x"]
        N, C, h = x.shape[1], x.shape[2], blk.heads
        M, Mq = B * N, B * Nq
        sq, skv = blk.stride_q[1], blk.stride_kv[1]
        thw, q_thw, k_thw = sv["thw"], sv["q_thw"], sv["k_thw"]
        self._red_slot = red_slot
        if red_begin:
            ops.reduce_defer(True)
        dy = dy.view(Mq, Co)
        dh = self._linear_bwd(dy, sv["act"], pre + "mlp.fc2.weight", pre + "mlp.fc2.bias", True,
                              epilogue=hip.EPI_DGELU, aux=sv["dact"])
        dxn2 = self._linear_bwd(dh, sv["xn2"].view(Mq, Co), pre + "mlp.fc1.weight",
                                pre + "mlp.fc1.bias", True, epilogue=hip.EPI_BF16)
        dx1, dy = ops.layernorm_bwd(dxn2, sv["x1"], f.p(pre + "norm2.weight"), sv["mean2"],
                                    sv["rstd2"], f.g(pre + "norm2.weight"), f.g(pre + "norm2.bias"),
                                    dres=dx2, want_bf16=True, row_scale=sv["dpa"], rows_per_sample=Nq,
                                    ws=self._rws("ln2"))
        dy = dy.view(Mq, Co)
        dctx = self._linear_bwd(dy, sv["ctx"].view(Mq, Co), pre + "attn.proj.weight",
                                pre + "attn.proj.bias", True, epilogue=hip.EPI_BF16)
        (qa, preq, mq, rq), (ka, prek, mk, rk), (v, prev, mv, rv) = sv["pools"]
        tabs, mats = sv["tabs"], sv["mats"]
        names = (pre + "attn.rel_pos_h", pre + "attn.rel_pos_w", pre + "attn.rel_pos_t")
        if all(m is None for m in mats):
            rcat_t, lpad, offs = f.rel_cat_t(pre)
        else:
            offs, lpad = rel_sections([t.shape[0] for t in tabs])
            rcat = torch.zeros((lpad, HD), device=self.dev, dtype=F32)
            for o, t in zip(offs, tabs):
                rcat[o:o + t.shape[0]] = t
            rcat_t = rcat.t().contiguous().to(BF16)
        if self.fused_scatter:
            dmap = self._relq_map(blk, q_thw, k_thw, sv["idx"], offs, n_obj, qa.shape[-1] - HD)
            dqa, dk, dv, D, dq_extra = ops.attn_bwd(
                qa, ka, v, sv["ctx"], dctx.view(B, Nq, Co), sv["lse2"], SCALE,
                q_splits=1 if self.deterministic else self.attn_q_splits, bias_cols=sum(sv["k_thw"]),
                reld=(dmap, lpad, LOG2E, rcat_t if rcat_t.is_contiguous() else None, "fold"))
        else:
            dqa, dk, dv = ops.attn_bwd(qa, ka, v, sv["ctx"], dctx.view(B, Nq, Co), sv["lse2"], SCALE,
                                       q_splits=1 if self.deterministic else self.attn_q_splits,
                                       bias_cols=sum(sv["k_thw"]))
            D = ops.relpos_scatter(dqa, sv["idx"], offs, lpad, B, h, q_thw, k_thw, n_obj, LOG2E)
            dq_extra = None
        qa2 = qa.view(B * h * Nq, qa.shape[-1])
        for n, m, t, o in zip(names, mats, tabs, offs):
            rows = t.shape[0]
            if m is None:
                self._tn.append((D[:, o:o + rows], qa2[:, :HD], f.g(n), None))
            else:
                d = torch.zeros_like(t)
                self._gemm_tn(D[:, o:o + rows], qa2[:, :HD], d)
                f.g(n).add_(m.t() @ d)
        if dq_extra is None:
            dq_extra = ops.gemm_nt(D, rcat_t, None, hip.EPI_BF16)
        elif isinstance(dq_extra, str):
            dq_extra = None
        Nk = ka.shape[2]
        dqkv = torch.empty_like(sv["qkv"])
        entries = []
        for r, pre_t, mean, rstd, nout, kw in (
                ("q", preq, mq, rq, Nq, dict(d_main=dqa, ld_main=qa.shape[-1], d_res=dctx,
                                             d_extra=dq_extra)),
                ("k", prek, mk, rk, Nk, dict(d_main=dk, ld_main=HD)),
                ("v", prev, mv, rv, Nk, dict(d_main=dv, ld_main=HD))):
            entries.append(((pre_t, mean, rstd, f.p(pre + "attn.norm_%s.weight" % r),
                             f.g(pre + "attn.norm_%s.weight" % r),
                             f.g(pre + "attn.norm_%s.bias" % r), B, h, nout), kw))
        dpres = ops.pool_ln_bwd_qkv(entries, ws=self._rws("pln"))
        strides = (sq, skv, skv)
        ops.pool_conv_bwd_qkv(dpres, [f.p(pre + "attn.pool_%s.weight" % r).view(HD, 27) for r in "qkv"],
                              dqkv, sv["qkv"],
                              [f.g(pre + "attn.pool_%s.weight" % r).view(HD, 27) for r in "qkv"],
                              B, h, thw, n_obj, strides, ws=self._wgrad_ws(B, h, thw, n_obj, strides))
        dxn = self._linear_bwd(dqkv, sv["xn"], pre + "attn.qkv.weight", pre + "attn.qkv.bias", True,
                               epilogue=hip.EPI_F32 if blk.has_proj else hip.EPI_BF16)
        dskip = dx1
        if blk.pools_q:
            dskip = ops.maxpool_bwd(dskip, sv["pool_idx"], thw, n_obj, bf16=blk.has_proj)
        if blk.has_proj:
            ds16 = dskip.view(M, Co) if blk.pools_q else ops.scale_cast(dskip.view(M, Co))
            self._linear_bwd(ds16, sv["xn"], pre + "proj.weight", pre + "proj.bias", True, out=dxn,
                             accumulate=True)
            dskip = None
        res = ops.layernorm_bwd(dxn, x, f.p(pre + "norm1.weight"), sv["mean1"], sv["rstd1"],
                                f.g(pre + "norm1.weight"), f.g(pre + "norm1.bias"), dres=dskip,
                                want_bf16=below is not None,
                                row_scale=below["dpm"] if below is not None else None,
                                rows_per_sample=N, ws=self._rws("ln1"))
        if red_end:
            ops.reduce_defer(False)
        self._flush_tn(force=False)
        if below is None:
            return res.view(B, N, C), None
        return res[0].view(B, N, C), res[1]
```

### svit_amd/hip.py

```python
import ctypes as C
import os

import torch

_HERE = os.path.dirname(os.path.abspath(__file__))
LIB_PATH = os.environ.get("SVIT_HIP_LIB") or os.path.join(_HERE, "lib", "libsvit_hip.so")
_lib = None

vp, i32, i64, f32 = C.c_void_p, C.c_int32, C.c_int64, C.c_float

EPI_BF16, EPI_GELU, EPI_RESID, EPI_F32, EPI_DGELU, EPI_RELQ = 0, 1, 2, 3, 4, 5


class TnProblem(C.Structure):
    _fields_ = [("A", vp), ("B", vp), ("dW", vp), ("dbias", vp), ("lda", i32), ("ldb", i32),
                ("lddw", i32), ("M", i32), ("N", i32), ("K", i32)]


class GemmArgs(C.Structure):
    _fields_ = [("A", vp), ("lda", i32), ("W", vp), ("ldw", i32), ("bias", vp), ("out", vp),
                ("ldo", i32), ("out2", vp), ("ldo2", i32), ("aux", vp), ("ldaux", i32),
                ("row_scale", vp), ("rows_per_sample", i32), ("M", i32), ("N", i32), ("K", i32),
                ("epilogue", i32), ("accumulate", i32), ("remap_L", i32), ("remap_N", i32),
                ("remap_off", i32), ("relq_map", vp), ("relq_out", vp), ("relq_ld", i32),
                ("relq_extra", i32), ("relq_rows", i32), ("relq_scale", f32)]


class PoolArgs(C.Structure):
    _fields_ = [("qkv", vp), ("which", i32), ("conv_w", vp), ("gamma", vp), ("beta", vp),
                ("out", vp), ("ld_out", i32), ("pre", vp), ("mean", vp), ("rstd", vp),
                ("B", i32), ("heads", i32), ("T", i32), ("H", i32), ("W", i32), ("n_obj", i32),
                ("stride_hw", i32), ("mode", i32), ("eps", f32), ("out_scale", f32),
                ("relq_R", vp), ("relq_map", vp), ("relq_lpad", i32), ("relq_scale", f32)]


class PoolLnBwdArgs(C.Structure):
    _fields_ = [("d_main", vp), ("main_is_f32", i32), ("ld_main", i32), ("d_res", vp),
                ("d_extra", vp), ("pre", vp), ("mean", vp), ("rstd", vp), ("gamma", vp),
                ("dpre", vp), ("dgamma", vp), ("dbeta", vp), ("B", i32), ("heads", i32),
                ("Nout", i32), ("workspace", vp), ("workspace_floats", i64), ("main_parts", i32),
                ("main_part_stride", i64), ("extra_is_bf16", i32)]


class PoolDgradArgs(C.Structure):
    _fields_ = [("dpre", vp), ("conv_w", vp), ("dqkv", vp), ("which", i32), ("B", i32),
                ("heads", i32), ("T", i32), ("H", i32), ("W", i32), ("n_obj", i32),
                ("stride_hw", i32)]


class PoolWgradArgs(C.Structure):
    _fields_ = [("dpre", vp), ("qkv", vp), ("which", i32), ("dw", vp), ("B", i32), ("heads", i32),
                ("T", i32), ("H", i32), ("W", i32), ("n_obj", i32), ("stride_hw", i32),
                ("workspace", vp), ("workspace_floats", i64)]


class RelqArgs(C.Structure):
    _fields_ = [("qa", vp), ("ld", i32), ("rel_h", vp), ("rel_w", vp), ("rel_t", vp),
                ("idx_h", vp), ("idx_w", vp), ("idx_t", vp), ("B", i32), ("heads", i32),
                ("qt", i32), ("qh", i32), ("qw", i32), ("kt", i32), ("kh", i32), ("kw", i32),
                ("n_obj", i32), ("inv_scale", f32)]


class RelqBwdArgs(C.Structure):
    _fields_ = [("qa", vp), ("dqa", vp), ("ld", i32), ("rel_h", vp), ("rel_w", vp), ("rel_t", vp),
                ("idx_h", vp), ("idx_w", vp), ("idx_t", vp), ("dq_extra", vp), ("drel_h", vp),
                ("drel_w", vp), ("drel_t", vp), ("rows_h", i32), ("rows_w", i32), ("rows_t", i32),
                ("B", i32), ("heads", i32), ("qt", i32), ("qh", i32), ("qw", i32), ("kt", i32),
                ("kh", i32), ("kw", i32), ("n_obj", i32), ("inv_scale", f32),
                ("workspace", vp), ("workspace_floats", i64)]


class RelqGatherArgs(C.Structure):
    _fields_ = [("P", vp), ("ldp", i32), ("qa", vp), ("ld", i32), ("idx_h", vp), ("idx_w", vp),
                ("idx_t", vp), ("row_h", i32), ("row_w", i32), ("row_t", i32), ("B", i32),
                ("heads", i32), ("qt", i32), ("qh", i32), ("qw", i32), ("kt", i32), ("kh", i32),
                ("kw", i32), ("n_obj", i32), ("inv_scale", f32)]


class RelqScatterArgs(C.Structure):
    _fields_ = [("dqa", vp), ("ld", i32), ("D", vp), ("ldd", i32), ("idx_h", vp), ("idx_w", vp),
                ("idx_t", vp), ("off_h", i32), ("off_w", i32), ("off_t", i32), ("B", i32),
                ("heads", i32), ("qt", i32), ("qh", i32), ("qw", i32), ("kt", i32), ("kh", i32),
                ("kw", i32), ("n_obj", i32), ("inv_scale", f32)]


class AttnFwdArgs(C.Structure):
    _fields_ = [("qa", vp), ("ka", vp), ("v", vp), ("ctx", vp), ("lse2", vp), ("B", i32),
                ("heads", i32), ("Nq", i32), ("Nk", i32), ("DA", i32), ("scale", f32),
                ("bias_cols", i32)]


class AttnBwdArgs(C.Structure):
    _fields_ = [("qa", vp), ("ka", vp), ("v", vp), ("ctx", vp), ("dctx", vp), ("lse2", vp),
                ("delta", vp), ("dqa", vp), ("dk", vp), ("dv", vp), ("B", i32), ("heads", i32),
                ("Nq", i32), ("Nk", i32), ("DA", i32), ("q_splits", i32), ("scale", f32),
                ("bias_cols", i32), ("relD", vp), ("relD_ld", i32), ("relD_map", vp), ("relD_scale", f32),
                ("relR", vp), ("relX", vp)]


class HeadArgs(C.Structure):
    _fields_ = [("tokens", vp), ("B", i32), ("N", i32), ("C", i32), ("T", i32), ("O", i32), ("keep", vp),
                ("w_proj", vp), ("b_proj", vp), ("n_cls", i32), ("w_box", vp), ("b_box", vp),
                ("w_bce", vp), ("b_bce", vp), ("w_con", vp), ("b_con", vp),
                ("logits", vp), ("boxes", vp), ("contact", vp), ("xobj", vp)]


class HeadBwdArgs(C.Structure):
    _fields_ = [("f", HeadArgs), ("dlogits", vp), ("dboxes", vp), ("dcontact", vp), ("dxobj", vp), ("dtokens", vp),
                ("gw_proj", vp), ("gb_proj", vp), ("gw_box", vp), ("gb_box", vp), ("gw_bce", vp), ("gb_bce", vp),
                ("gw_con", vp), ("gb_con", vp), ("ordered", i32)]


class StepHost(C.Structure):
    _fields_ = [("lr", f32 * 2), ("weight_decay", f32 * 2), ("max_norm", f32), ("clip_value", f32),
                ("grad_scale", f32), ("reserved", f32)]


class StepDev(C.Structure):
    _fields_ = [("applied", i64), ("skipped", i64), ("consecutive", i32), ("apply", i32), ("coef", f32),
                ("bc1", f32), ("bc2_sqrt", f32), ("sumsq", f32), ("grad_norm", f32), ("reserved", f32)]


_SIGS = {
    "svit_version": (i32, []),
    "svit_arch": (C.c_char_p, []),
    "svit_gemm_nt": (i32, [C.POINTER(GemmArgs), vp]),
    "svit_gemm_tn": (i32, [vp, i32, vp, i32, vp, i32, i32, i32, i32, i32, vp, vp]),
    "svit_gemm_tn_grouped": (i32, [C.POINTER(TnProblem), i32, vp]),
    "svit_gemm_tn_grouped_ex": (i32, [C.POINTER(TnProblem), i32, i32, vp]),
    "svit_gemm_tn_grouped_slab": (i32, [C.POINTER(TnProblem), i32, vp, i64, vp]),
    "svit_gemm_tn_grouped_workspace": (i64, [C.POINTER(TnProblem), i32]),
    "svit_colsum_bf16": (i32, [vp, i32, vp, i32, i32, vp]),
    "svit_cast_f32_bf16": (i32, [vp, vp, i64, vp]),
    "svit_table_interp": (i32, [vp, i32, i32, vp, vp, vp, vp]),
    "svit_table_interp_batched": (i32, [vp, i32, i32, vp]),
    "svit_transpose_cast_batched": (i32, [vp, vp, vp, i32, i32, vp]),
    "svit_transpose_bf16_batched": (i32, [vp, vp, vp, i32, i32, vp]),
    "svit_scale_cast": (i32, [vp, vp, vp, i32, i64, i32, i32, i32, i32, vp]),
    "svit_pad_cast_rows": (i32, [vp, vp, i32, i32, i32, vp]),
    "svit_reduce_defer": (i32, [i32, vp]),
    "svit_reduce_flush": (i32, [vp]),
    "svit_reduce_reset": (i32, [vp]),
    "svit_layernorm_fwd": (i32, [vp, vp, vp, vp, vp, vp, vp, i64, i32, f32, vp]),
    "svit_layernorm_bwd": (i32, [vp, i32, vp, vp, vp, vp, vp, vp, vp, vp, i32, vp, vp, i64, i32, vp,
                                 i64, vp]),
    "svit_im2col_patch": (i32, [vp, vp, i32, i32, i32, i32, vp]),
    "svit_im2col_patch_u8": (i32, [vp, i64, vp, vp, vp, i32, i32, i32, i32, i32, vp]),
    "svit_im2col_patch_u8_mix": (i32, [vp, i64, vp, vp, vp, vp, i32, i32, i32, i32, i32, vp]),
    "svit_mixup_clips": (i32, [vp, vp, i32, i32, i32, i32, vp]),
    "svit_fill_special_tokens": (i32, [vp, vp, vp, vp, i32, i32, i32, i32, i32, i32, i32, vp]),
    "svit_special_token_grads": (i32, [vp, vp, vp, vp, i32, i32, i32, i32, i32, i32, i32, vp]),
    "svit_pool_ln_fwd": (i32, [C.POINTER(PoolArgs), vp]),
    "svit_pool_ln_bwd": (i32, [C.POINTER(PoolLnBwdArgs), vp]),
    "svit_pool_ln_fwd_qkv": (i32, [C.POINTER(PoolArgs), vp]),
    "svit_pool_ln_fwd_qkv_sel": (i32, [C.POINTER(PoolArgs), C.POINTER(vp), vp]),
    "svit_pool_weight_sel": (i32, [vp, vp, vp, i32, vp]),
    "svit_pool_ln_bwd_qkv": (i32, [C.POINTER(PoolLnBwdArgs), vp]),
    "svit_pool_conv_bwd_qkv": (i32, [C.POINTER(PoolDgradArgs), C.POINTER(PoolWgradArgs), vp]),
    "svit_pool_conv_bwd_workspace": (i64, [C.POINTER(PoolDgradArgs)]),
    "svit_relpos_q_fwd": (i32, [C.POINTER(RelqArgs), vp]),
    "svit_relpos_q_bwd": (i32, [C.POINTER(RelqBwdArgs), vp]),
    "svit_relpos_scatter": (i32, [C.POINTER(RelqScatterArgs), vp]),
    "svit_relpos_gather": (i32, [C.POINTER(RelqGatherArgs), vp]),
    "svit_attn_fwd": (i32, [C.POINTER(AttnFwdArgs), vp]),
    "svit_attn_bwd": (i32, [C.POINTER(AttnBwdArgs), vp]),
    "svit_attn_bwd_parts": (i32, [C.POINTER(AttnBwdArgs)]),
    "svit_maxpool_fwd": (i32, [vp, vp, vp, i32, i32, i32, i32, i32, i32, vp]),
    "svit_maxpool_bwd": (i32, [vp, vp, vp, i32, i32, i32, i32, i32, i32, vp]),
    "svit_maxpool_bwd_bf16": (i32, [vp, vp, vp, i32, i32, i32, i32, i32, i32, vp]),
    "svit_sumsq": (i32, [vp, i64, vp, vp, i64, vp]),
    "svit_adamw_step": (i32, [vp, vp, vp, vp, i64, vp, f32, f32, f32, f32, f32, f32, i32, f32, vp]),
    "svit_adamw_bias_table": (i32, [f32, f32, vp, i64, C.POINTER(i64)]),
    "svit_step_guard": (i32, [vp, i64, vp, vp, vp, i64, vp, i64, vp]),
    "svit_adamw_step_guarded": (i32, [vp, vp, vp, vp, i64, i64, vp, vp, f32, f32, f32, vp]),
    "svit_head_fwd": (i32, [C.POINTER(HeadArgs), vp]),
    "svit_head_bwd": (i32, [C.POINTER(HeadBwdArgs), vp]),
    "svit_haog_loss": (i32, [vp, vp, vp, vp, vp, vp, vp, vp, vp, i32, i32, vp]),
    "svit_haog_loss_bwd": (i32, [vp, vp, vp, vp, vp, vp, vp, i32, i32, vp]),
    "svit_ce_loss": (i32, [vp, vp, i32, i32, vp, vp, vp]),
    "svit_ce_loss_soft": (i32, [vp, vp, vp, vp, f32, f32, i32, i32, vp, vp, vp]),
# ... 92 lines not shown
```

### svit_amd/ops.py

```python
import ctypes as C

import torch

from . import hip
from .hip import ptr

BF16 = torch.bfloat16
F32 = torch.float32
HD = 96
_scratch = {}


def scratch(device, floats=8 * 1024 * 1024, tag="main"):
    key = (device.index, floats, tag)
    buf = _scratch.get(key)
    if buf is None:
        buf = torch.empty(floats, device=device, dtype=F32)
        _scratch[key] = buf
    return buf


def _chk_rows(*ts):
    for t in ts:
        if not t.is_cuda or t.dim() != 2 or t.stride(1) != 1:
# ... 442 lines not shown
    a.workspace, a.workspace_floats = ptr(ws), ws.numel()




def pool_conv_bwd_workspace(B, heads, thw, n_obj, strides):
    da = (hip.PoolDgradArgs * 3)()
    for i in range(3):
        da[i].B, da[i].heads, (da[i].T, da[i].H, da[i].W), da[i].n_obj, da[i].stride_hw, da[i].which = B, heads, thw, n_obj, strides[i], i
    return int(hip.load().svit_pool_conv_bwd_workspace(da))


def pool_conv_bwd_qkv(dpres, conv_ws, dqkv, qkv, dws, B, heads, thw, n_obj, strides, ws=None):
    if ws is None:
        need = pool_conv_bwd_workspace(B, heads, thw, n_obj, strides)
        ws = scratch(dpres[0].device, max(8 * 1024 * 1024, need), tag="poolbwd")
    da = (hip.PoolDgradArgs * 3)()
    wa = (hip.PoolWgradArgs * 3)()
    for i in range(3):
        _pool_dgrad_args(da[i], dpres[i], conv_ws[i], dqkv, i, B, heads, thw, n_obj, strides[i])
        _pool_wgrad_args(wa[i], dpres[i], qkv, i, dws[i], B, heads, thw, n_obj, strides[i], ws)
    hip.call("svit_pool_conv_bwd_qkv", da, wa)


def relpos_q_fwd(qa, tabs, idx, B, heads, q_thw, k_thw, n_obj, inv_scale):
    a = hip.RelqArgs()
    a.qa, a.ld = ptr(qa), qa.shape[-1]
    a.rel_h, a.rel_w, a.rel_t = (ptr(t) for t in tabs)
    a.idx_h, a.idx_w, a.idx_t = (ptr(t) for t in idx)
    a.B, a.heads = B, heads
    a.qt, a.qh, a.qw = q_thw
    a.kt, a.kh, a.kw = k_thw
    a.n_obj, a.inv_scale = n_obj, inv_scale
    hip.call("svit_relpos_q_fwd", C.byref(a))


def relpos_q_bwd(qa, dqa, tabs, idx, dtabs, B, heads, q_thw, k_thw, n_obj, inv_scale):
    Nq = qa.shape[2]
    dq_extra = torch.empty((B, heads, Nq, HD), device=qa.device, dtype=F32)
    a = hip.RelqBwdArgs()
    a.qa, a.dqa, a.ld = ptr(qa), ptr(dqa), qa.shape[-1]
    a.rel_h, a.rel_w, a.rel_t = (ptr(t) for t in tabs)
    a.idx_h, a.idx_w, a.idx_t = (ptr(t) for t in idx)
    a.dq_extra = ptr(dq_extra)
    a.drel_h, a.drel_w, a.drel_t = (ptr(t) for t in dtabs)
    a.rows_h, a.rows_w, a.rows_t = (t.shape[0] for t in tabs)
    a.B, a.heads = B, heads
    a.qt, a.qh, a.qw = q_thw
    a.kt, a.kh, a.kw = k_thw
    a.n_obj, a.inv_scale = n_obj, inv_scale
    ws = scratch(qa.device)
    a.workspace, a.workspace_floats = ptr(ws), ws.numel()
    hip.call("svit_relpos_q_bwd", C.byref(a))
    return dq_extra


def relpos_gather(P, qa, idx, rows_off, B, heads, q_thw, k_thw, n_obj, inv_scale):
    a = hip.RelqGatherArgs()
    a.P, a.ldp, a.qa, a.ld = ptr(P), P.shape[-1], ptr(qa), qa.shape[-1]
    a.idx_h, a.idx_w, a.idx_t = (ptr(t) for t in idx)
    a.row_h, a.row_w, a.row_t = rows_off
    a.B, a.heads = B, heads
    a.qt, a.qh, a.qw = q_thw
    a.kt, a.kh, a.kw = k_thw
    a.n_obj, a.inv_scale = n_obj, inv_scale
    hip.call("svit_relpos_gather", C.byref(a))


def relpos_scatter(dqa, idx, offs, ldd, B, heads, q_thw, k_thw, n_obj, inv_scale):
    Nq = dqa.shape[2]
    D = torch.empty((B * heads * Nq, ldd), device=dqa.device, dtype=BF16)
    a = hip.RelqScatterArgs()
    a.dqa, a.ld, a.D, a.ldd = ptr(dqa), dqa.shape[-1], ptr(D), ldd
    a.idx_h, a.idx_w, a.idx_t = (ptr(t) for t in idx)
    a.off_h, a.off_w, a.off_t = offs
    a.B, a.heads = B, heads
    a.qt, a.qh, a.qw = q_thw
    a.kt, a.kh, a.kw = k_thw
    a.n_obj, a.inv_scale = n_obj, inv_scale
    hip.call("svit_relpos_scatter", C.byref(a))
    return D


def attn_fwd(qa, ka, v, scale, bias_cols=0):
    _chk_dev(qa, ka, v)
    B, heads, Nq, DA = qa.shape
    Nk = ka.shape[2]
    ctx = torch.empty((B, Nq, heads * HD), device=qa.device, dtype=BF16)
    lse2 = torch.empty((B, heads, Nq), device=qa.device, dtype=F32)
    a = hip.AttnFwdArgs()
    a.qa, a.ka, a.v, a.ctx, a.lse2 = ptr(qa), ptr(ka), ptr(v), ptr(ctx), ptr(lse2)
    a.B, a.heads, a.Nq, a.Nk, a.DA, a.scale, a.bias_cols = B, heads, Nq, Nk, DA, scale, bias_cols
    hip.call("svit_attn_fwd", C.byref(a), meta=("attn", B, heads, Nq, Nk, DA))
    return ctx, lse2


def attn_bwd(qa, ka, v, ctx, dctx, lse2, scale, q_splits=0, bias_cols=0, reld=None):
    _chk_dev(qa, ka, v, ctx, dctx, lse2)
    B, heads, Nq, DA = qa.shape
    Nk = ka.shape[2]
    dev = qa.device
    a = hip.AttnBwdArgs()
    a.B, a.heads, a.Nq, a.Nk, a.DA, a.q_splits, a.scale = B, heads, Nq, Nk, DA, q_splits, scale
    a.bias_cols = bias_cols
    parts = hip.load().svit_attn_bwd_parts(C.byref(a))
    if parts < 1:
        raise hip.SvitHipError("svit_attn_bwd_parts failed: %d" % parts)
    dqa = torch.empty((B, heads, Nq, DA), device=dev, dtype=BF16)
    dkv = torch.empty((2, parts, B, heads, Nk, HD), device=dev, dtype=F32)
    delta = torch.empty((B, heads, Nq, 2), device=dev, dtype=F32)
    a.qa, a.ka, a.v, a.ctx, a.dctx, a.lse2 = (ptr(t) for t in (qa, ka, v, ctx, dctx, lse2))
    a.delta, a.dqa, a.dk, a.dv = ptr(delta), ptr(dqa), ptr(dkv[0]), ptr(dkv[1])
    a.q_splits = parts
    D = X = None
    if reld is not None:
        cmap, ldd, rscale = reld[:3]
        rt = reld[3] if len(reld) > 3 else None
        _chk_dev(cmap, rt)
        assert cmap.dtype == torch.int32 and cmap.is_contiguous() and cmap.shape == (Nq, DA - HD)
        D = torch.empty((B * heads * Nq, ldd), device=dev, dtype=BF16)
        a.relD, a.relD_ld, a.relD_map, a.relD_scale = ptr(D), ldd, ptr(cmap), rscale
        mode = reld[4] if len(reld) > 4 else "separate"
        if rt is not None and ldd <= 128 and ldd % 16 == 0:
            assert rt.dtype == BF16 and rt.is_contiguous() and tuple(rt.shape) == (HD, ldd)
            a.relR = ptr(rt)
            if mode == "fold":
                X = "folded"
            else:
                X = torch.empty((B * heads * Nq, HD), device=dev, dtype=F32)
                a.relX = ptr(X)
    folded = 2.0 * B * heads * Nq * HD * reld[1] if (reld is not None and X is not None) else 0.0
    hip.call("svit_attn_bwd", C.byref(a), meta=("attn", B, heads, Nq, Nk, DA, folded))
    if reld is not None:
        return dqa, dkv[0], dkv[1], D, X
    return dqa, dkv[0], dkv[1]


def maxpool_fwd(x, thw, n_obj):
    B, N, C_ = x.shape
    T, H, W = thw
    Nout = 1 + T * pooled(H, 2) * pooled(W, 2) + n_obj
    y = torch.empty((B, Nout, C_), device=x.device, dtype=F32)
    idx = torch.empty((B, Nout, C_), device=x.device, dtype=torch.uint8)
    hip.call("svit_maxpool_fwd", ptr(x), ptr(y), ptr(idx), B, T, H, W, n_obj, C_)
    return y, idx


def maxpool_bwd(dy, idx, thw, n_obj, bf16=False):
    B, Nout, C_ = dy.shape
    T, H, W = thw
    dx = torch.empty((B, 1 + T * H * W + n_obj, C_), device=dy.device, dtype=BF16 if bf16 else F32)
    hip.call("svit_maxpool_bwd_bf16" if bf16 else "svit_maxpool_bwd", ptr(dy), ptr(idx), ptr(dx),
             B, T, H, W, n_obj, C_)
    return dx


def sumsq(g, out):
    ws = scratch(g.device)
    hip.call("svit_sumsq", ptr(g), g.numel(), ptr(out), ptr(ws), ws.numel())


def adamw_step(p, g, m, v, sumsq_t, max_norm, lr, beta1, beta2, eps, wd, step, grad_scale=1.0):
    hip.call("svit_adamw_step", ptr(p), ptr(g), ptr(m), ptr(v), p.numel(), ptr(sumsq_t), max_norm,
             lr, beta1, beta2, eps, wd, step, grad_scale)


def adamw_bias_table(beta1, beta2):
    import numpy as np
    cap = 1 << 20
    buf = np.empty((cap, 2), dtype=np.float32)
    n = C.c_int64(0)
    rc = hip.load().svit_adamw_bias_table(beta1, beta2, buf.ctypes.data, cap, C.byref(n))
    hip.check(rc, "svit_adamw_bias_table (betas %r, %r)" % (beta1, beta2))
    return buf[:n.value].copy()


def _chk_step_records(host_rec, dev_rec, device):
    _chk_dev(host_rec, dev_rec)
    if (host_rec.dtype != F32 or host_rec.numel() != 8 or dev_rec.dtype != torch.int32 or dev_rec.numel() != 12
            or host_rec.device != device or dev_rec.device != device):
        raise hip.SvitHipError("the step record is fp32 [8] + int32 [12] on %s" % (device,))


def step_guard(g, host_rec, dev_rec, table, workspace):
    _chk_dev(g, table, workspace)
    _chk_step_records(host_rec, dev_rec, g.device)
    hip.call("svit_step_guard", ptr(g), g.numel(), ptr(host_rec), ptr(dev_rec), ptr(table), table.shape[0],
             ptr(workspace), workspace.numel())


def adamw_step_guarded(p, g, m, v, n_decay, host_rec, dev_rec, beta1, beta2, eps):
    _chk_dev(p, g, m, v)
    _chk_step_records(host_rec, dev_rec, p.device)
    n = p.numel()
    if g.numel() != n or m.numel() != n or v.numel() != n:
        raise hip.SvitHipError("adamw_step_guarded: p, g, m, v differ in size")
# ... 106 lines not shown
```

Baseline: 698.5 clips/s.

## Skip attention and GEMM work for drop-path-dead samples

Passes the per-sample drop-path scale into the attention forward/backward kernels and the NT GEMMs. Workgroups whose sample has scale zero write zeros to their outputs and exit without the main loop. This removes compute for samples dropped by stochastic depth, at the cost of a per-tile branch and reliance on those branch outputs being truly unused. It is enabled by default through a new knob.

```diff
diff --git a/include/svit_hip.h b/include/svit_hip.h
--- a/include/svit_hip.h
+++ b/include/svit_hip.h
@@ -186,6 +186,7 @@
 typedef struct {
   const void* qa; const void* ka; const void* v; void* ctx; float* lse2;
   int32_t B, heads, Nq, Nk, DA; float scale; int32_t bias_cols;
+  const float* sample_scale;
 } svit_attn_fwd_args;
 int svit_attn_fwd(const svit_attn_fwd_args* a, void* stream);
 typedef struct {
@@ -197,6 +198,7 @@
   int32_t bias_cols;
   void* relD; int32_t relD_ld; const int32_t* relD_map; float relD_scale;
   const void* relR; float* relX;
+  const float* sample_scale;
 } svit_attn_bwd_args;
 int svit_attn_bwd(const svit_attn_bwd_args* a, void* stream);
 int svit_attn_bwd_parts(const svit_attn_bwd_args* a);
diff --git a/svit_amd/csrc/attn_bwd.hip b/svit_amd/csrc/attn_bwd.hip
--- a/svit_amd/csrc/attn_bwd.hip
+++ b/svit_amd/csrc/attn_bwd.hip
@@ -60,6 +60,15 @@
   const int q0 = qtile * 128 + wave * 32;
   const int qi = q0 + (lane & 31);
   const int qc = min(qi, a.Nq - 1);
+  if (sample_dead(a.sample_scale, b)) {
+    const int r0 = qtile * 128, r1 = min(r0 + 128, a.Nq);
+    zero_rows((bf16_t*)a.dqa + ((size_t)bh * a.Nq) * DA, (size_t)DA * 2, DA / 8, r0, r1, tid, 256);
+    if (a.relD) zero_rows((bf16_t*)a.relD + ((size_t)bh * a.Nq) * a.relD_ld, (size_t)a.relD_ld * 2, a.relD_ld >> 3, r0, r1, tid, 256);
+    if (a.relX) zero_rows(a.relX + ((size_t)bh * a.Nq) * HD, (size_t)HD * 4, HD / 4, r0, r1, tid, 256);
+    float* sc = a.delta + (size_t)bh * a.Nq * 2;
+    for (int i = r0 + tid; i < r1; i += 256) { sc[i] = 0.f; sc[a.Nq + i] = 0.f; }
+    return;
+  }
   const bf16_t* qa = (const bf16_t*)a.qa + ((size_t)bh * a.Nq) * DA;
   const bf16_t* ka = (const bf16_t*)a.ka + ((size_t)bh * a.Nk) * DA;
   const bf16_t* vv = (const bf16_t*)a.v + ((size_t)bh * a.Nk) * HD;
@@ -373,6 +382,13 @@
   const int key0 = bx * 128;
   const int ki = key0 + kg * 32 + (lane & 31);
   const int kc = min(ki, a.Nk - 1);
+  if (sample_dead(a.sample_scale, b)) {
+    const size_t row0 = ((size_t)by * a.B * a.heads + bh) * a.Nk;
+    const int r1 = min(key0 + 128, a.Nk);
+    zero_rows(a.dk + row0 * HD, (size_t)HD * 4, HD / 4, key0, r1, tid, 256 * NH);
+    zero_rows(a.dv + row0 * HD, (size_t)HD * 4, HD / 4, key0, r1, tid, 256 * NH);
+    return;
+  }
   const bf16_t* qa = (const bf16_t*)a.qa + ((size_t)bh * a.Nq) * DA;
   const bf16_t* ka = (const bf16_t*)a.ka + ((size_t)bh * a.Nk) * DA;
   const bf16_t* vv = (const bf16_t*)a.v + ((size_t)bh * a.Nk) * HD;
@@ -642,6 +658,9 @@
   const int bias_cols = a->bias_cols > 0 ? a->bias_cols : a->DA - 96;
   const int ksu = 6 + (bias_cols + 15) / 16;
   hipStream_t st = (hipStream_t)stream;
-  if (a->DA == 128) return ksu <= 7 ? launch_bwd<128, 7>(*a, st) : launch_bwd<128, 8>(*a, st);
-  return ksu <= 9 ? launch_bwd<160, 9>(*a, st) : launch_bwd<160, 10>(*a, st);
-}
+  svit_attn_bwd_args copy = *a;
+  if (!(svit_knob(SVIT_K_DROP_SKIP) & 1)) copy.sample_scale = nullptr;
+  if (copy.sample_scale && (((uintptr_t)copy.relX | (uintptr_t)copy.dk | (uintptr_t)copy.dv) & 15)) return SVIT_ERR_ALIGN;
+  if (a->DA == 128) return ksu <= 7 ? launch_bwd<128, 7>(copy, st) : launch_bwd<128, 8>(copy, st);
+  return ksu <= 9 ? launch_bwd<160, 9>(copy, st) : launch_bwd<160, 10>(copy, st);
+}
diff --git a/svit_amd/csrc/attn_common.h b/svit_amd/csrc/attn_common.h
--- a/svit_amd/csrc/attn_common.h
+++ b/svit_amd/csrc/attn_common.h
@@ -349,6 +349,14 @@
   asm volatile("s_waitcnt vmcnt(%0)" ::"n"(N) : "memory");
 }
 
+__device__ __forceinline__ bool sample_dead(const float* sample_scale, int b) {
+  return sample_scale != nullptr && sample_scale[b] == 0.0f;
+}
+__device__ __forceinline__ void zero_rows(void* base, size_t ld_bytes, int cpr, int r0, int r1, int tid, int nthreads) {
+  const int n = (r1 - r0) * cpr;
+  for (int i = tid; i < n; i += nthreads)
+    *(uint4*)((unsigned char*)base + (size_t)(r0 + i / cpr) * ld_bytes + (size_t)(i % cpr) * 16) = make_uint4(0u, 0u, 0u, 0u);
+}
 }
 
 
diff --git a/svit_amd/csrc/attn_fwd.hip b/svit_amd/csrc/attn_fwd.hip
--- a/svit_amd/csrc/attn_fwd.hip
+++ b/svit_amd/csrc/attn_fwd.hip
@@ -57,6 +57,12 @@
   const int q0 = (wgid % gridDim.x) * (NW * 32) + wave * 32;
   const int qi = q0 + (lane & 31);
   const int qc = min(qi, a.Nq - 1);
+  if (sample_dead(a.sample_scale, b)) {
+    const int r0 = (wgid % gridDim.x) * (NW * 32), r1 = min(r0 + NW * 32, a.Nq);
+    zero_rows((bf16_t*)a.ctx + ((size_t)b * a.Nq) * a.heads * HD + head * HD, (size_t)a.heads * HD * 2, 12, r0, r1, tid, NW * 64);
+    for (int i = r0 + tid; i < r1; i += NW * 64) a.lse2[(size_t)bh * a.Nq + i] = 0.f;
+    return;
+  }
   const bf16_t* qa = (const bf16_t*)a.qa + ((size_t)bh * a.Nq) * DA;
   const bf16_t* ka = (const bf16_t*)a.ka + ((size_t)bh * a.Nk) * DA;
   const bf16_t* vv = (const bf16_t*)a.v + ((size_t)bh * a.Nk) * HD;
@@ -291,6 +297,12 @@
   const int bh = wgid / gridDim.x, b = bh / a.heads, head = bh % a.heads;
   const int ntiles = (a.Nq + 127) / 128;
   const int t_begin = (wgid % gridDim.x) * tiles_per_wg, t_end = min(ntiles, t_begin + tiles_per_wg);
+  if (sample_dead(a.sample_scale, b)) {
+    const int r0 = t_begin * 128, r1 = min(t_end * 128, a.Nq);
+    zero_rows((bf16_t*)a.ctx + ((size_t)b * a.Nq) * a.heads * HD + head * HD, (size_t)a.heads * HD * 2, 12, r0, r1, tid, 256);
+    for (int i = r0 + tid; i < r1; i += 256) a.lse2[(size_t)bh * a.Nq + i] = 0.f;
+    return;
+  }
   const bf16_t* qa = (const bf16_t*)a.qa + ((size_t)bh * a.Nq) * DA;
   const bf16_t* ka = (const bf16_t*)a.ka + ((size_t)bh * a.Nk) * DA;
   const bf16_t* vv = (const bf16_t*)a.v + ((size_t)bh * a.Nk) * HD;
@@ -494,8 +506,12 @@
   return wide ? launch_cfg<KSU, 8, 3>(a, st) : launch_cfg<KSU, 4, 2>(a, st);
 }
 }
-extern "C" int svit_attn_fwd(const svit_attn_fwd_args* a, void* stream) {
-  if (!a || !a->qa || !a->ka || !a->v || !a->ctx || !a->lse2) return SVIT_ERR_ARG;
+extern "C" int svit_attn_fwd(const svit_attn_fwd_args* args, void* stream) {
+  if (!args) return SVIT_ERR_ARG;
+  svit_attn_fwd_args copy = *args;
+  if (!(svit_knob(SVIT_K_DROP_SKIP) & 1)) copy.sample_scale = nullptr;
+  const svit_attn_fwd_args* a = &copy;
+  if (!a->qa || !a->ka || !a->v || !a->ctx || !a->lse2) return SVIT_ERR_ARG;
   if (a->B <= 0 || a->heads <= 0 || a->Nq <= 0 || a->Nk <= 0) return SVIT_ERR_SHAPE;
   if (((uintptr_t)a->qa | (uintptr_t)a->ka | (uintptr_t)a->v | (uintptr_t)a->ctx) & 15)
     return SVIT_ERR_ALIGN;
diff --git a/svit_amd/csrc/common.h b/svit_amd/csrc/common.h
--- a/svit_amd/csrc/common.h
+++ b/svit_amd/csrc/common.h
@@ -42,6 +42,7 @@
   SVIT_K_ATTN_DKV_FORM,
   SVIT_K_ATTN_FWD_SHORT,
   SVIT_K_POOL_FRAME,
+  SVIT_K_DROP_SKIP,
   SVIT_K_COUNT
 };
 int svit_knob(int k);
diff --git a/svit_amd/csrc/gemm_nt.hip b/svit_amd/csrc/gemm_nt.hip
--- a/svit_amd/csrc/gemm_nt.hip
+++ b/svit_amd/csrc/gemm_nt.hip
@@ -14,9 +14,17 @@
   asm volatile("s_waitcnt vmcnt(%0)" ::"n"(N) : "memory");
 }
 
+__device__ __forceinline__ bool nt_tile_dead(const svit_gemm_args& p, int skip, int m0, int BM) {
+  if (!skip) return false;
+  const int s_last = (min(m0 + BM, p.M) - 1) / p.rows_per_sample;
+  bool dead = true;
+  for (int s = m0 / p.rows_per_sample; s <= s_last; ++s) dead = dead && p.row_scale[s] == 0.0f;
+  return dead;
+}
+
 template <int RB, int NB, int WAVES_M, int WAVES_N, int STAGES, int EPI, int BK2>
 __global__ __launch_bounds__(WAVES_M* WAVES_N * 64, (WAVES_M * WAVES_N > 4 ? 1 : 2)) void
-gemm_nt_v2_kernel(svit_gemm_args p) {
+gemm_nt_v2_kernel(svit_gemm_args p, int skip) {
   constexpr int NT = WAVES_M * WAVES_N * 64;
   constexpr int BM = 32 * RB * WAVES_M, WN = 32 * NB, BN = WN * WAVES_N;
   constexpr int CPR = BK2 / 8;
@@ -71,7 +79,7 @@
 #pragma unroll
       for (int r = 0; r < 16; ++r) acc[i][j][r] = 0.f;
 
-  const int nk = p.K / BK2;
+  const int nk = nt_tile_dead(p, skip, m0, BM) ? 0 : p.K / BK2;
 #pragma unroll
   for (int s = 0; s < STAGES - 1; ++s)
     if (s < nk) issue(s, s);
@@ -110,6 +118,10 @@
   }
   __syncthreads();
   nt_epilogue<RB, NB, EPI, true>(p, acc, smem, m0, n0, wm, wn, lane, wave);
+}
+
+static inline int nt_skip(const svit_gemm_args& a) {
+  return a.row_scale && a.rows_per_sample > 0 && a.epilogue != SVIT_EPI_RELQ && (svit_knob(SVIT_K_DROP_SKIP) & 2) ? 1 : 0;
 }
 
 template <int RB, int NB, int WAVES_M, int WAVES_N, int STAGES, int BK2 = 32>
@@ -131,7 +143,7 @@
 #define SVIT_V2_CASE(E)                                                                       \
   case E:                                                                                     \
     hipLaunchKernelGGL((gemm_nt_v2_kernel<RB, NB, WAVES_M, WAVES_N, STAGES, E, BK2>), grid, dim3(NT), \
-                       lds, st, a);                                                           \
+                       lds, st, a, nt_skip(a));                                               \
     break;
   switch (a.epilogue) {
     SVIT_V2_CASE(SVIT_EPI_BF16)
@@ -185,7 +197,7 @@
 }
 
 template <int RB, int NB, int WAVES_M, int WAVES_N, int NL, int STAGES, int EPI>
-__global__ __launch_bounds__((WAVES_M * WAVES_N + NL) * 64, 1) void gemm_nt_ring_kernel(svit_gemm_args p) {
+__global__ __launch_bounds__((WAVES_M * WAVES_N + NL) * 64, 1) void gemm_nt_ring_kernel(svit_gemm_args p, int skip) {
   using attn::Int;
   constexpr int NC = WAVES_M * WAVES_N;
   constexpr int BM = 32 * RB * WAVES_M, WN = 32 * NB, BN = WN * WAVES_N;
@@ -199,7 +211,7 @@
   const int xq = nwg >> 3, xr = nwg & 7, xcd = lin & 7;
   const int wgid = (xcd < xr ? xcd * (xq + 1) : xr * (xq + 1) + (xcd - xr) * xq) + (lin >> 3);
   const int m0 = (wgid / gridDim.x) * BM, n0 = (wgid % gridDim.x) * BN;
-  const int nk = p.K / 64;
+  const int nk = nt_tile_dead(p, skip, m0, BM) ? 0 : p.K / 64;
 
   if (wave >= NC) {
     nt_ring_loader<NL, BM, BN, STAGES>(p, smem, wave - NC, lane, m0, n0, nk);
@@ -252,9 +264,11 @@
     });
   };
 
-  __builtin_amdgcn_s_barrier();
-  attn::static_for<0, NH>([&](auto H) { reads(Int<0>{}, Int<0>{}, 0u, H); });
-  release(Int<0>{});
+  if (nk > 0) {
+    __builtin_amdgcn_s_barrier();
+    attn::static_for<0, NH>([&](auto H) { reads(Int<0>{}, Int<0>{}, 0u, H); });
+    release(Int<0>{});
+  }
   for (int kt = 0; kt < nk; ++kt) {
     const unsigned so = (unsigned)((kt % STAGES) * STAGE_BYTES);
     const unsigned so_next = (unsigned)(((kt + 1) % STAGES) * STAGE_BYTES);
@@ -289,7 +303,7 @@
 #undef SVIT_RING_ATTR
 #define SVIT_RING_CASE(E)                                                                       \
   case E:                                                                                       \
-    hipLaunchKernelGGL((gemm_nt_ring_kernel<RB, NB, WAVES_M, WAVES_N, NL, STAGES, E>), grid, dim3(NT), lds, st, a); \
+    hipLaunchKernelGGL((gemm_nt_ring_kernel<RB, NB, WAVES_M, WAVES_N, NL, STAGES, E>), grid, dim3(NT), lds, st, a, nt_skip(a)); \
     break;
   switch (a.epilogue) {
     SVIT_RING_CASE(SVIT_EPI_BF16)
@@ -333,7 +347,8 @@
   if (a.aux && (a.ldaux % 4 != 0 || ((uintptr_t)a.aux & 15))) return SVIT_ERR_ALIGN;
   if (a.out2 && (a.ldo2 % 4 != 0 || ((uintptr_t)a.out2 & 15))) return SVIT_ERR_ALIGN;
   if ((a.epilogue == SVIT_EPI_RESID || a.epilogue == SVIT_EPI_DGELU) && !a.aux) return SVIT_ERR_ARG;
-  if (a.epilogue == SVIT_EPI_RESID && a.row_scale && a.rows_per_sample <= 0) return SVIT_ERR_ARG;
+  if (a.row_scale && a.rows_per_sample <= 0) return SVIT_ERR_ARG;
+  if (a.row_scale && a.epilogue == SVIT_EPI_F32 && a.remap_L > 0) return SVIT_ERR_ARG;
   hipStream_t st = (hipStream_t)stream;
   const int force_raw = svit_knob(SVIT_K_NT_CFG), force_stages = svit_knob(SVIT_K_NT_STAGES);
   const bool no_ring = force_raw == 8 || svit_knob(SVIT_K_NT_BK) != 0;
diff --git a/svit_amd/csrc/misc.hip b/svit_amd/csrc/misc.hip
--- a/svit_amd/csrc/misc.hip
+++ b/svit_amd/csrc/misc.hip
@@ -569,8 +569,9 @@
 
 static const int k_knob_default[SVIT_K_COUNT] = {
      0,  -1,  0,  85,  75,  2,
-     2,  1,  1,  0,  1,  2};
-static int g_knob[SVIT_K_COUNT] = {0, -1, 0, 85, 75, 2, 2, 1, 1, 0, 1, 2};
+     2,  1,  1,  0,  1,  2,
+     3};
+static int g_knob[SVIT_K_COUNT] = {0, -1, 0, 85, 75, 2, 2, 1, 1, 0, 1, 2, 3};
 int svit_knob(int k) { return __atomic_load_n(&g_knob[k], __ATOMIC_RELAXED); }
 int svit_knob_set(int k, int v) {
   if (k < 0 || k >= SVIT_K_COUNT) return SVIT_ERR_ARG;
@@ -584,6 +585,7 @@
   if (key == 0) return (val == 0 || (val >= 2 && val <= 4)) ? svit_knob_set(SVIT_K_NT_STAGES, val) : SVIT_ERR_ARG;
   if (key == 1) return (val >= -1 && val <= 10) ? svit_knob_set(SVIT_K_NT_CFG, val) : SVIT_ERR_ARG;
   if (key == 2) return (val == 0 || val == 32 || val == 64) ? svit_knob_set(SVIT_K_NT_BK, val) : SVIT_ERR_ARG;
+  if (key == 3) return (val >= 0 && val <= 3) ? svit_knob_set(SVIT_K_DROP_SKIP, val) : SVIT_ERR_ARG;
   return SVIT_ERR_ARG;
 }
 extern "C" int svit_debug_set_tn(int step_us_x100, int atomic_tbs_x100) {
diff --git a/svit_amd/engine.py b/svit_amd/engine.py
--- a/svit_amd/engine.py
+++ b/svit_amd/engine.py
@@ -309,7 +309,9 @@
         xn, _, mean1, rstd1 = ops.layernorm_fwd(x, f.p(pre + "norm1.weight"), f.p(pre + "norm1.bias"),
                                                 save_stats=save)
         xn2d = xn.view(B * N, C)
-        qkv = ops.gemm_nt(xn2d, f.w(pre + "attn.qkv.weight"), f.p(pre + "attn.qkv.bias"), hip.EPI_BF16)
+        dpa, dpm = ds if ds is not None else (None, None)
+        qkv = ops.gemm_nt(xn2d, f.w(pre + "attn.qkv.weight"), f.p(pre + "attn.qkv.bias"), hip.EPI_BF16,
+                          row_scale=dpa, rows_per_sample=N)
         idx, mats, mcat, need = self._rel(blk, q_thw, k_thw)
         if mcat is None:
             tabs = self._tables(pre, mats)
@@ -331,7 +333,7 @@
             else None,
             relq=(rcat.contiguous(), self._relq_map(blk, q_thw, k_thw, idx, rows_off, n_obj, DA - HD), LOG2E))
         qa, ka, v = pools[0][0], pools[1][0], pools[2][0]
-        ctx, lse2 = ops.attn_fwd(qa, ka, v, SCALE, bias_cols=J)
+        ctx, lse2 = ops.attn_fwd(qa, ka, v, SCALE, bias_cols=J, sample_scale=dpa)
         pool_idx = None
         if blk.has_proj:
             skip = ops.gemm_nt(xn2d, f.w(pre + "proj.weight"), f.p(pre + "proj.bias"), hip.EPI_F32)
@@ -340,14 +342,13 @@
             skip = x
         if blk.pools_q:
             skip, pool_idx = ops.maxpool_fwd(skip, thw, n_obj)
-        dpa, dpm = ds if ds is not None else (None, None)
         x1 = ops.gemm_nt(ctx.view(B * Nq, Co), f.w(pre + "attn.proj.weight"), f.p(pre + "attn.proj.bias"),
                          hip.EPI_RESID, aux=skip.view(B * Nq, Co), row_scale=dpa, rows_per_sample=Nq)
         x1 = x1.view(B, Nq, Co)
         xn2, _, mean2, rstd2 = ops.layernorm_fwd(x1, f.p(pre + "norm2.weight"), f.p(pre + "norm2.bias"),
                                                  save_stats=save)
         act, dact = ops.gemm_nt(xn2.view(B * Nq, Co), f.w(pre + "mlp.fc1.weight"),
-                                f.p(pre + "mlp.fc1.bias"), hip.EPI_GELU, save=save)
+                                f.p(pre + "mlp.fc1.bias"), hip.EPI_GELU, save=save, row_scale=dpm, rows_per_sample=Nq)
         x2 = ops.gemm_nt(act, f.w(pre + "mlp.fc2.weight"), f.p(pre + "mlp.fc2.bias"), hip.EPI_RESID,
                          aux=x1.view(B * Nq, Co), row_scale=dpm, rows_per_sample=Nq).view(B, Nq, Co)
         sv = None
@@ -463,12 +464,14 @@
             ops.gemm_tn(a, b, dw, splits=0, dbias=dbias)
 
     def _linear_bwd(self, dy16, x16, wname, bname, need_dx, out=None, accumulate=False,
-                    epilogue=hip.EPI_F32, aux=None):
+                    epilogue=hip.EPI_F32, aux=None, dead=None):
         f = self.flat
         self._tn.append((dy16, x16, f.g(wname), f.g(bname)))
         if not need_dx:
             return None
-        return ops.gemm_nt(dy16, f.wt(wname), None, epilogue, out=out, aux=aux, accumulate=accumulate)
+        rs, rps = dead if dead is not None and dead[0] is not None else (None, 0)
+        return ops.gemm_nt(dy16, f.wt(wname), None, epilogue, out=out, aux=aux, accumulate=accumulate,
+                           row_scale=rs, rows_per_sample=rps)
 
     def _block_bwd(self, blk, sv, dx2, dy, n_obj, below, red_begin=True, red_end=True, red_slot=0):
         f = self.flat
@@ -484,16 +487,17 @@
             ops.reduce_defer(True)
         dy = dy.view(Mq, Co)
         dh = self._linear_bwd(dy, sv["act"], pre + "mlp.fc2.weight", pre + "mlp.fc2.bias", True,
-                              epilogue=hip.EPI_DGELU, aux=sv["dact"])
+                              epilogue=hip.EPI_DGELU, aux=sv["dact"], dead=(sv["dpm"], Nq))
         dxn2 = self._linear_bwd(dh, sv["xn2"].view(Mq, Co), pre + "mlp.fc1.weight",
-                                pre + "mlp.fc1.bias", True, epilogue=hip.EPI_BF16)
+                                pre + "mlp.fc1.bias", True, epilogue=hip.EPI_BF16,
+                                dead=(sv["dpm"], Nq))
         dx1, dy = ops.layernorm_bwd(dxn2, sv["x1"], f.p(pre + "norm2.weight"), sv["mean2"],
                                     sv["rstd2"], f.g(pre + "norm2.weight"), f.g(pre + "norm2.bias"),
                                     dres=dx2, want_bf16=True, row_scale=sv["dpa"], rows_per_sample=Nq,
                                     ws=self._rws("ln2"))
         dy = dy.view(Mq, Co)
         dctx = self._linear_bwd(dy, sv["ctx"].view(Mq, Co), pre + "attn.proj.weight",
-                                pre + "attn.proj.bias", True, epilogue=hip.EPI_BF16)
+                                pre + "attn.proj.bias", True, epilogue=hip.EPI_BF16, dead=(sv["dpa"], Nq))
         (qa, preq, mq, rq), (ka, prek, mk, rk), (v, prev, mv, rv) = sv["pools"]
         tabs, mats = sv["tabs"], sv["mats"]
         names = (pre + "attn.rel_pos_h", pre + "attn.rel_pos_w", pre + "attn.rel_pos_t")
@@ -510,11 +514,11 @@
             dqa, dk, dv, D, dq_extra = ops.attn_bwd(
                 qa, ka, v, sv["ctx"], dctx.view(B, Nq, Co), sv["lse2"], SCALE,
                 q_splits=1 if self.deterministic else self.attn_q_splits, bias_cols=sum(sv["k_thw"]),
-                reld=(dmap, lpad, LOG2E, rcat_t if rcat_t.is_contiguous() else None, "fold"))
+                reld=(dmap, lpad, LOG2E, rcat_t if rcat_t.is_contiguous() else None, "fold"), sample_scale=sv["dpa"])
         else:
             dqa, dk, dv = ops.attn_bwd(qa, ka, v, sv["ctx"], dctx.view(B, Nq, Co), sv["lse2"], SCALE,
                                        q_splits=1 if self.deterministic else self.attn_q_splits,
-                                       bias_cols=sum(sv["k_thw"]))
+                                       bias_cols=sum(sv["k_thw"]), sample_scale=sv["dpa"])
             D = ops.relpos_scatter(dqa, sv["idx"], offs, lpad, B, h, q_thw, k_thw, n_obj, LOG2E)
             dq_extra = None
         qa2 = qa.view(B * h * Nq, qa.shape[-1])
@@ -548,7 +552,7 @@
                               [f.g(pre + "attn.pool_%s.weight" % r).view(HD, 27) for r in "qkv"],
                               B, h, thw, n_obj, strides, ws=self._wgrad_ws(B, h, thw, n_obj, strides))
         dxn = self._linear_bwd(dqkv, sv["xn"], pre + "attn.qkv.weight", pre + "attn.qkv.bias", True,
-                               epilogue=hip.EPI_F32 if blk.has_proj else hip.EPI_BF16)
+                               epilogue=hip.EPI_F32 if blk.has_proj else hip.EPI_BF16, dead=(sv["dpa"], N))
         dskip = dx1
         if blk.pools_q:
             dskip = ops.maxpool_bwd(dskip, sv["pool_idx"], thw, n_obj, bf16=blk.has_proj)
diff --git a/svit_amd/hip.py b/svit_amd/hip.py
--- a/svit_amd/hip.py
+++ b/svit_amd/hip.py
@@ -87,7 +87,7 @@
 class AttnFwdArgs(C.Structure):
     _fields_ = [("qa", vp), ("ka", vp), ("v", vp), ("ctx", vp), ("lse2", vp), ("B", i32),
                 ("heads", i32), ("Nq", i32), ("Nk", i32), ("DA", i32), ("scale", f32),
-                ("bias_cols", i32)]
+                ("bias_cols", i32), ("sample_scale", vp)]
 
 
 class AttnBwdArgs(C.Structure):
@@ -95,7 +95,7 @@
                 ("delta", vp), ("dqa", vp), ("dk", vp), ("dv", vp), ("B", i32), ("heads", i32),
                 ("Nq", i32), ("Nk", i32), ("DA", i32), ("q_splits", i32), ("scale", f32),
                 ("bias_cols", i32), ("relD", vp), ("relD_ld", i32), ("relD_map", vp), ("relD_scale", f32),
-                ("relR", vp), ("relX", vp)]
+                ("relR", vp), ("relX", vp), ("sample_scale", vp)]
 
 
 class HeadArgs(C.Structure):
diff --git a/svit_amd/ops.py b/svit_amd/ops.py
--- a/svit_amd/ops.py
+++ b/svit_amd/ops.py
@@ -548,8 +548,8 @@
     return D
 
 
-def attn_fwd(qa, ka, v, scale, bias_cols=0):
-    _chk_dev(qa, ka, v)
+def attn_fwd(qa, ka, v, scale, bias_cols=0, sample_scale=None):
+    _chk_dev(qa, ka, v, sample_scale)
     B, heads, Nq, DA = qa.shape
     Nk = ka.shape[2]
     ctx = torch.empty((B, Nq, heads * HD), device=qa.device, dtype=BF16)
@@ -557,12 +557,13 @@
     a = hip.AttnFwdArgs()
     a.qa, a.ka, a.v, a.ctx, a.lse2 = ptr(qa), ptr(ka), ptr(v), ptr(ctx), ptr(lse2)
     a.B, a.heads, a.Nq, a.Nk, a.DA, a.scale, a.bias_cols = B, heads, Nq, Nk, DA, scale, bias_cols
+    a.sample_scale = ptr(sample_scale)
     hip.call("svit_attn_fwd", C.byref(a), meta=("attn", B, heads, Nq, Nk, DA))
     return ctx, lse2
 
 
-def attn_bwd(qa, ka, v, ctx, dctx, lse2, scale, q_splits=0, bias_cols=0, reld=None):
-    _chk_dev(qa, ka, v, ctx, dctx, lse2)
+def attn_bwd(qa, ka, v, ctx, dctx, lse2, scale, q_splits=0, bias_cols=0, reld=None, sample_scale=None):
+    _chk_dev(qa, ka, v, ctx, dctx, lse2, sample_scale)
     B, heads, Nq, DA = qa.shape
     Nk = ka.shape[2]
     dev = qa.device
@@ -578,6 +579,7 @@
     a.qa, a.ka, a.v, a.ctx, a.dctx, a.lse2 = (ptr(t) for t in (qa, ka, v, ctx, dctx, lse2))
     a.delta, a.dqa, a.dk, a.dv = ptr(delta), ptr(dqa), ptr(dkv[0]), ptr(dkv[1])
     a.q_splits = parts
+    a.sample_scale = ptr(sample_scale)
     D = X = None
     if reld is not None:
         cmap, ldd, rscale = reld[:3]
```

Result: slower. 691.5 clips/s (-1.0%).
